# vinayak-gholap1993/Geometric-Multigrid-preconditioners-for-long-range-Coulomb-interaction

Hardware: AMD Instinct MI355X
Metric: DoF/s per CG-iter (GMG-precond Poisson, 3D) (higher is better)
Workload: dtype f64

## Files before the change

geometric-multigrid-preconditioners-for-long-range-coulomb-interaction_amd/capi.py:

```python
from __future__ import annotations

import ctypes as C
import os

import numpy as np

from . import build as _build

OK, ERR_INVALID, ERR_OUTER_NOCONV, ERR_COARSE_NOCONV, ERR_HIP, ERR_COMM, ERR_UNSUPPORTED = range(7)
SYSTEM = -1
JACOBI, SSOR, CHEBYSHEV = 0, 1, 2
PRECOND_GMG, PRECOND_JACOBI, PRECOND_IDENTITY = 0, 1, 2
SSOR_PARTITION_ROWS, SSOR_PARTITION_BALANCED = 0, 1
COARSE_CG, COARSE_DIRECT = 0, 1
CHEB_FIRST_KIND, CHEB_FOURTH_KIND = 0, 1
CHEB_LMAX_GERSHGORIN, CHEB_LMAX_LANCZOS = 0, 1
CHEBYSHEV_KEYS = ("polynomial", "lmax_source", "lanczos_steps", "steps_run", "gershgorin", "ritz", "safety", "lmax")
LEVEL_A, LEVEL_EDGE, LEVEL_EDGE_T = 0, 1, 2
UNIQUE_ID_BYTES = 128

SYMBOLS = [
    "gmg_create", "gmg_destroy", "gmg_reset", "gmg_last_error", "gmg_synchronize",
    "gmg_set_system_matrix", "gmg_set_level_matrix", "gmg_set_level_matrix_lattice", "gmg_set_edge_matrix", "gmg_set_prolongation", "gmg_build_transfer", "gmg_get_transfer",
    "gmg_assemble_system_matrix", "gmg_get_system_matrix", "gmg_system_matrix_norms",
    "gmg_assemble_level_matrix", "gmg_get_level_matrix", "gmg_assemble_system_matrix_coef", "gmg_assemble_level_matrix_coef",
    "gmg_assemble_rhs", "gmg_distribute_constraints",
    "gmg_build_mesh_tables", "gmg_get_mesh_tables", "gmg_get_mesh_level_tables",
    "gmg_close_constraints", "gmg_get_closed_constraints",
    "gmg_assemble_system_matrix_resident", "gmg_assemble_system_matrix_coef_resident", "gmg_assemble_level_matrix_resident",
    "gmg_assemble_level_matrix_coef_resident", "gmg_assemble_rhs_resident", "gmg_distribute_constraints_resident",
    "gmg_refine_forest", "gmg_get_refined_forest", "gmg_transfer_solution", "gmg_build_face_table",
    "gmg_estimate_error",
    "gmg_build_face_table_resident", "gmg_get_face_table", "gmg_estimate_error_resident", "gmg_get_marks", "gmg_refine_forest_marked",
    "gmg_energy_norm_error_resident",
    "gmg_build_point_locator_resident", "gmg_get_point_locator", "gmg_atom_forces_resident", "gmg_electrostatic_energy_resident",
    "gmg_set_copy_indices", "gmg_set_smoother", "gmg_set_coarse", "gmg_set_chebyshev", "gmg_estimate_lmax", "gmg_get_chebyshev",
    "gmg_set_coarse_solver", "gmg_coarse_direct_tables", "gmg_coarse_direct_separable", "gmg_coarse_direct_transform", "gmg_coarse_direct_profile",
    "gmg_vec_alloc", "gmg_vec_free", "gmg_vec_upload", "gmg_vec_download", "gmg_vec_set_zero", "gmg_vec_equ",
    "gmg_vec_add", "gmg_vec_sadd", "gmg_vec_dot", "gmg_vec_norms", "gmg_vec_all_zero",
    "gmg_spmv", "gmg_precondition", "gmg_precondition_jacobi", "gmg_coarse_solve", "gmg_smoother_step",
    "gmg_prolongate", "gmg_restrict_and_add", "gmg_cg_solve", "gmg_cg_direction_step", "gmg_cg_update_step",
    "gmg_comm_unique_id", "gmg_comm_init", "gmg_comm_barrier", "gmg_comm_info", "gmg_set_halo_plan", "gmg_set_global_sizes", "gmg_partition_range",
    "gmg_vec_allgather",
    "gmg_stats_reset", "gmg_stats_get", "gmg_set_profiling", "gmg_set_tuning", "gmg_set_option", "gmg_set_ssor_blocks",
    "gmg_set_ssor_block_rows", "gmg_set_ssor_partition", "gmg_get_ssor_partition", "gmg_ssor_balance_rows", "gmg_calibrate_hbm", "gmg_charge_density", "gmg_get_charge_density", "gmg_rhs_assemble",
    "gmg_charge_density_resident", "gmg_get_resident_cell_geometry",
    "gmg_set_point_locator", "gmg_atom_forces", "gmg_direct_coulomb",
    "gmg_gaussian_potential", "gmg_energy_norm_error",
    "gmg_get_ssor_plan", "gmg_get_ssor_backward_rows", "gmg_ssor_slot_plan",
    "gmg_get_ssor_plan_array", "gmg_get_ssor_plan_origin",
]


class Stats(C.Structure):
    _fields_ = [("coarse_solves", C.c_int64), ("coarse_iterations", C.c_int64), ("vcycles", C.c_int64),
                ("spmv0_samples", C.c_int64), ("spmv0_ms_total", C.c_double), ("spmv0_rows", C.c_int64),
                ("spmv0_nnz", C.c_int64), ("cgupd_samples", C.c_int64), ("cgupd_ms_total", C.c_double),
                ("coarse_variant", C.c_int64), ("spmv0_layout", C.c_int64), ("spmv0_matrix_bytes", C.c_int64),
                ("spmv0_pattern_slices", C.c_int64), ("spmv0_slices", C.c_int64), ("coarse_enqueued", C.c_int64),
                ("spmv0_noop_samples", C.c_int64), ("spmv0_noop_ms_total", C.c_double),
                ("sgs_samples", C.c_int64), ("sgs_ms_total", C.c_double), ("sgs_substeps", C.c_int64), ("sgs_stream_bytes", C.c_int64),
                ("sgs_launches", C.c_int64), ("build_matrices_ms", C.c_double), ("coarse_solver", C.c_int64)]


class GMGError(RuntimeError):
    def __init__(self, code, msg):
        super().__init__(f"gmg error {code}: {msg}")
        self.code = code


_lib = None


def load(build_if_missing: bool = False):
    global _lib
    if _lib is None:
        path = os.environ.get("GMG_DEVICE_LIB") or _build.LIB_DEVICE
        if build_if_missing:
            _build.build_device()
        if not os.path.exists(path):
            raise FileNotFoundError(f"{path} missing: run __graft_entry__.build() (hipcc --offload-arch=gfx950)")
        _lib = C.CDLL(path)
        _lib.gmg_last_error.restype = C.c_char_p
        _lib.gmg_last_error.argtypes = [C.c_void_p]
    return _lib


def _p(a, t):
    return a.ctypes.data_as(C.POINTER(t))


def _csr(m):
    return (np.ascontiguousarray(m.rowptr, dtype=np.int64), np.ascontiguousarray(m.col, dtype=np.int32),
            np.ascontiguousarray(m.val, dtype=np.float64))


class DeviceVector:
    def __init__(self, ctx: "Context", n: int):
        self.ctx, self.n = ctx, int(n)
        self.ptr = C.POINTER(C.c_double)()
        ctx._chk(ctx.L.gmg_vec_alloc(ctx.h, C.c_int64(self.n), C.byref(self.ptr)))

    def upload(self, a):
        a = np.ascontiguousarray(a, dtype=np.float64)
        assert a.size == self.n
        self.ctx._chk(self.ctx.L.gmg_vec_upload(self.ctx.h, self.ptr, _p(a, C.c_double), C.c_int64(self.n)))
        return self

    def download(self):
        out = np.empty(self.n)
        self.ctx._chk(self.ctx.L.gmg_vec_download(self.ctx.h, _p(out, C.c_double), self.ptr, C.c_int64(self.n)))
        return out

    def free(self):
        if self.ptr:
            self.ctx.L.gmg_vec_free(self.ctx.h, self.ptr)
            self.ptr = C.POINTER(C.c_double)()


class Context:

    def __init__(self, n_levels: int, device: int = 0):
        self.L = load()
        self.h = C.c_void_p()
        rc = self.L.gmg_create(C.byref(self.h), C.c_int(device), C.c_int(n_levels))
        if rc != OK:
            raise GMGError(rc, "gmg_create failed (no MI355X visible?)")
        self.n_levels = n_levels
        self.n_system = 0

    @classmethod
    def view(cls, handle):
        self = cls.__new__(cls)
# ... 789 lines not shown
    def synchronize(self):
        self._chk(self.L.gmg_synchronize(self.h))

    @staticmethod
    def unique_id() -> bytes:
        buf = C.create_string_buffer(UNIQUE_ID_BYTES)
        rc = load().gmg_comm_unique_id(buf)
        if rc != OK:
            raise GMGError(rc, "gmg_comm_unique_id failed")
        return buf.raw

    def comm_init(self, rank, n_ranks, uid: bytes):
        buf = C.create_string_buffer(uid, UNIQUE_ID_BYTES)
        self._chk(self.L.gmg_comm_init(self.h, C.c_int(rank), C.c_int(n_ranks), buf))

    def comm_barrier(self):
        self._chk(self.L.gmg_comm_barrier(self.h))

    def comm_info(self) -> dict:
        out = (C.c_int64 * 8)()
        self._chk(self.L.gmg_comm_info(self.h, out))
        return {"ranks": int(out[0]), "transport": {0: "none", 1: "rccl", 2: "peer"}[int(out[1])], "mailbox_finegrained": bool(out[2]),
                "ring_memory": {-1: "not allocated", 0: "hipMalloc (coarse-grained)", 1: "fine-grained"}[int(out[3])],
                "devices": int(out[4]), "level0_partitioned": bool(out[5])}

    def set_global_sizes(self, n_system, n_level0):
        self._chk(self.L.gmg_set_global_sizes(self.h, C.c_int64(n_system), C.c_int64(n_level0)))

    def allgather(self, n_global, dst_full, src_local):
        self._chk(self.L.gmg_vec_allgather(self.h, C.c_int64(n_global), dst_full.ptr, src_local.ptr))

    def set_halo_plan(self, which, neighbor_rank, send_count, send_idx, recv_count):
        nr = np.ascontiguousarray(neighbor_rank, dtype=np.int32)
        sc = np.ascontiguousarray(send_count, dtype=np.int32)
        si = np.ascontiguousarray(send_idx, dtype=np.int32)
        rc_ = np.ascontiguousarray(recv_count, dtype=np.int32)
        self._chk(self.L.gmg_set_halo_plan(self.h, C.c_int(which), C.c_int(len(nr)), _p(nr, C.c_int32), _p(sc, C.c_int32),
                                           _p(si, C.c_int32), _p(rc_, C.c_int32)))

    def stats(self) -> Stats:
        s = Stats()
        self._chk(self.L.gmg_stats_get(self.h, C.byref(s)))
        return s

    def stats_reset(self):
        self._chk(self.L.gmg_stats_reset(self.h))

    def set_profiling(self, every):
        self._chk(self.L.gmg_set_profiling(self.h, C.c_int(every)))

    def calibrate_hbm(self, n_bytes=1 << 30, reps=10):
        r, c = C.c_double(0), C.c_double(0)
        self._chk(self.L.gmg_calibrate_hbm(self.h, C.c_int64(n_bytes), C.c_int(reps), C.byref(r), C.byref(c)))
        return r.value, c.value

    def set_tuning(self, coarse_chunk=0, cg_variant=0, ssor_blocks=0):
        self._chk(self.L.gmg_set_tuning(self.h, C.c_int(coarse_chunk), C.c_int(cg_variant)))
        if ssor_blocks:
            self._chk(self.L.gmg_set_ssor_blocks(self.h, C.c_int(ssor_blocks)))

    def set_option(self, key: str, value: float = 1.0):
        self._chk(self.L.gmg_set_option(self.h, key.encode(), C.c_double(value)))

    def set_ssor_block_rows(self, level, block_row):
        b = np.ascontiguousarray(block_row, dtype=np.int64)
        n_blocks = max(len(b) - 1, 0)
        self._chk(self.L.gmg_set_ssor_block_rows(self.h, C.c_int(level), C.c_int(n_blocks), _p(b, C.c_int64) if len(b) else None))

    def set_ssor_partition(self, kind):
        self._chk(self.L.gmg_set_ssor_partition(self.h, C.c_int(kind)))

    def get_ssor_partition(self, level):
        nb = C.c_int(0)
        self._chk(self.L.gmg_get_ssor_partition(self.h, C.c_int(level), C.byref(nb), None, None))
        br, st = np.zeros(nb.value + 1, dtype=np.int64), np.zeros(max(nb.value, 1), dtype=np.int64)
        self._chk(self.L.gmg_get_ssor_partition(self.h, C.c_int(level), C.byref(nb), _p(br, C.c_int64), _p(st, C.c_int64)))
        return br, st[:nb.value]

    def get_ssor_plan(self, level):
        out = np.zeros(8, dtype=np.int64)
        self._chk(self.L.gmg_get_ssor_plan(self.h, C.c_int(level), _p(out, C.c_int64)))
        return dict(zip(SSOR_PLAN_KEYS, (int(v) for v in out)))

    def get_ssor_backward_rows(self, level):
        cnt = C.c_int64(0)
        self._chk(self.L.gmg_get_ssor_backward_rows(self.h, C.c_int(level), C.byref(cnt), None))
        rows = np.zeros(max(cnt.value, 1), dtype=np.int32)
        self._chk(self.L.gmg_get_ssor_backward_rows(self.h, C.c_int(level), C.byref(cnt), _p(rows, C.c_int32)))
        return rows[:cnt.value]

    def get_ssor_plan_array(self, level, which):
        w = SSOR_PLAN_ARRAYS.index(which) if isinstance(which, str) else int(which)
        nbytes = C.c_int64(0)
        self._chk(self.L.gmg_get_ssor_plan_array(self.h, C.c_int(level), C.c_int(w), C.byref(nbytes), None))
        out = np.zeros(max(nbytes.value, 1), dtype=np.uint8)
        self._chk(self.L.gmg_get_ssor_plan_array(self.h, C.c_int(level), C.c_int(w), C.byref(nbytes), out.ctypes.data_as(C.c_void_p)))
        return out[:nbytes.value]

    def get_ssor_plan_origin(self, level):
        on_dev, moved, why = C.c_int(0), C.c_int64(0), C.c_char_p()
        self._chk(self.L.gmg_get_ssor_plan_origin(self.h, C.c_int(level), C.byref(on_dev), C.byref(moved), C.byref(why)))
        return bool(on_dev.value), int(moved.value), (why.value or b"").decode()


SSOR_PLAN_ARRAYS = ("stream", "ranges", "blk_tab", "block_rng", "row_ci", "ci_row", "rpos_f", "rpos_b", "iso_diag", "iso_invd")
SSOR_PLAN_KEYS = ("forward_ranges", "backward_ranges", "self_contained_ranges", "y_slots", "max_live_forward", "max_live_backward", "steps", "stream_bytes")


def ssor_slot_plan(m, row_begin, row_end, backward):
    rp, col, val = _csr(m)
    n = len(rp) - 1
    k = max(int(row_end) - int(row_begin), 1)
    step, last, slot = (np.full(k, -1, dtype=np.int32) for _ in range(3))
    ns, nl = C.c_int64(0), C.c_int64(0)
    rc = load().gmg_ssor_slot_plan(C.c_int64(n), _p(rp, C.c_int64), _p(col, C.c_int32), _p(val, C.c_double), C.c_int64(int(row_begin)), C.c_int64(int(row_end)),
                                   C.c_int(int(bool(backward))), _p(step, C.c_int32), _p(last, C.c_int32), _p(slot, C.c_int32), C.byref(ns), C.byref(nl))
    if rc != OK:
        raise GMGError(rc, "gmg_ssor_slot_plan")
    k = int(row_end) - int(row_begin)
    return step[:k], last[:k], slot[:k], ns.value, nl.value


def ssor_balance_rows(m, n_blocks, use_values=True):
    rp, col, val = _csr(m)
    n = len(rp) - 1
    br, cost = np.zeros(n_blocks + 1, dtype=np.int64), np.zeros(n_blocks)
    rc = load().gmg_ssor_balance_rows(C.c_int64(n), _p(rp, C.c_int64), _p(col, C.c_int32), _p(val, C.c_double) if use_values else None,
                                      C.c_int(n_blocks), _p(br, C.c_int64), _p(cost, C.c_double))
    if rc != OK:
        raise GMGError(rc, "gmg_ssor_balance_rows")
    return br, cost


def coarse_direct_tables(n_cells):
    m = int(n_cells) - 1
    S, lam, mu = np.zeros((max(m, 1), max(m, 1))), np.zeros(max(m, 1)), np.zeros(max(m, 1))
    rc = load().gmg_coarse_direct_tables(C.c_int(int(n_cells)), _p(S, C.c_double), _p(lam, C.c_double), _p(mu, C.c_double))
    if rc != OK:
        raise GMGError(rc, "gmg_coarse_direct_tables")
    return S, lam, mu


def coarse_direct_separable(Ke):
    ke = np.ascontiguousarray(Ke, dtype=np.float64).reshape(64)
    s = C.c_double(0)
    rc = load().gmg_coarse_direct_separable(_p(ke, C.c_double), C.byref(s))
    if rc == ERR_UNSUPPORTED:
        return None
    if rc != OK:
        raise GMGError(rc, "gmg_coarse_direct_separable")
    return s.value
```

geometric-multigrid-preconditioners-for-long-range-coulomb-interaction_amd/csrc/gmg_coulomb.hip:

```cpp
#include "../../include/gmg_coulomb.h"
#include "gmg_device.hpp"
#include "gmg_sgs_layout.hpp"
#include "gmg_sgs.hpp"
#include "gmg_sgs_phase.hpp"
#include "gmg_sgs_dep.hpp"
#include "gmg_sgs_reg.hpp"
#include "gmg_sgs_plan.hpp"
#ifdef GMG_EXPERIMENTS
#include "gmg_sgs_chain.hpp"
#endif
#include "gmg_lattice.hpp"
#include "gmg_transfer.hpp"
#include "gmg_forces.hpp"
#include "gmg_exact.hpp"
#include "gmg_assemble.hpp"
#include "gmg_rhs_cells.hpp"
#include "gmg_estimate.hpp"
#include "gmg_fastdiag.hpp"
#include "gmg_lanczos.hpp"
#include "gmg_mesh_tables.hpp"
#include "gmg_close.hpp"
#include "gmg_refine.hpp"
#include "gmg_density.hpp"
#include "gmg_mem.hpp"
#include <hip/hip_ext.h>

#include <algorithm>
#include <array>
#include <chrono>
#include <cmath>
#include <cstdio>
#include <cstdlib>
#include <cstring>
#include <climits>
#include <map>
#include <queue>
#include <string>
#include <thread>
#include <unordered_map>
#include <vector>

#include "gmg_comm.hpp"

using namespace gmg;

namespace {

struct DevCSR {
  int64_t n_rows = 0, n_cols = 0, nnz = 0;
  DevPtr<int32_t> rowptr, col;
  DevPtr<double> val;
  DevPtr<int32_t> tile_row;
  int n_tiles = 0, tiles_per_xcd = 0, grid = 0;
  bool valid = false;
  HaloPlan halo;
  bool sell = false;
  DevPtr<int32_t> slice_ptr;
  DevPtr<int32_t> slice_base;
  DevPtr<void> sell_vals;
  DevPtr<void> sell_cols;
  DevPtr<double> sell_dict;
  DevPtr<int32_t> sell_spat, sell_pat;
  int sellp_pid = -1, sellp_centre[9] = {};
  DevPtr<int32_t> sellp_wave_ptr;
  DevPtr<int4> sellp_wave_rr;
  bool use_sellp = false;
  bool rowclass = false;
  DevPtr<uint8_t> sellp_rowcls;
  DevPtr<double> sellp_ctab;
  int n_classes = 0;
  int n_patterns = 0, n_pattern_slices = 0;
  bool val8 = false, col16 = false;
  int n_slices = 0, sell_grid = 0;
  int64_t sell_quads = 0;
  bool lattice = false;
  DevPtr<uint8_t> lat_rowcls;
  DevPtr<double> lat_ctab;
  DevPtr<int32_t> lat_gen;
  bool lat_only = false;
  int lat_W = 0;
  int64_t lat_fast_rows = 0;
  int lat_classes = 0, lat_nx = 0, lat_nxy = 0, lat_R0 = 0, lat_R1 = 0, lat_C = 0, lat_K = 0, lat_S = 0, lat_fast_blocks = 0, lat_n_gen = 0, lat_grid = 0;
  int64_t lat_gen_bytes = 0;
  bool hyb = false, hyb_val8 = false;
  DevPtr<int32_t> hyb_qptr, hyb_spat, hyb_pat, hyb_tiles, hyb_reg;
  DevPtr<void> hyb_vals, hyb_cols;
  DevPtr<double> hyb_dict;
  int hyb_n_slices = 0, hyb_n_reg = 0, hyb_n_pattern_slices = 0, hyb_n_tiles = 0, hyb_tile_blocks = 0, hyb_grid = 0;
  int64_t hyb_stream_bytes = 0, hyb_csr_bytes = 0;
  int lat_nv[3] = {0, 0, 0};
  double lat_Ke[64] = {};
};

struct SgsPlan {
  DevPtr<int32_t> stage_ptr, stage_rows, block_row, block_stage;
  int n_blocks = 0;
  int n_stages_max = 0;
  bool wave = false;
  DevPtr<SwRange> w_ranges;
  DevPtr<int32_t> w_block_rng, w_ws_ci, w_ci_row, w_row_ci, w_rpos_f, w_rpos_b;
  DevPtr<char> w_stream;
  DevPtr<double> w_ycur, w_iso_diag, w_iso_invd;
  int w_y_slots = 0, w_lds_bytes = 0, w_n_ranges = 0;
  int n_bwd = 0;
  std::vector<int32_t> host_bwd_rows;
  int n_self = 0, live_max[2] = {0, 0};
  int64_t w_n_coupled = 0, w_stream_bytes = 0, w_steps = 0, w_stages = 0;
  std::vector<int32_t> host_block_row;
  std::vector<int64_t> host_block_steps;
  std::vector<int64_t> host_block_bytes;
  std::vector<int32_t> host_block_rng;
  DevPtr<double> w_stage;
  int64_t w_stage_len = 0;
  bool phased = false;
  bool dep = false;
  bool reg = false;
  DevPtr<PhRange> p_ranges;
  DevPtr<uint4> p_blk_tab;
  std::vector<PhRange> host_pranges;
  bool on_device = false;
  int64_t csr_bytes_down = 0;
  const char *host_reason = "";
};

struct Level {
  DevCSR A, I, It, P, Pt;
  bool has_I = false, has_P = false;
  int64_t n = 0;
  int64_t n_vec = 0;
  int64_t n_copy = 0;
  DevPtr<int32_t> copy_g, copy_l;
  std::vector<int32_t> host_copy_g, host_copy_l;
  int copy_version = 0;
  DevPtr<double> sol, def, t, w1, w2, w3;
  double *sol_full = nullptr, *def_full = nullptr;
  DevPtr<double> sol_full_own, def_full_own;
  DevPtr<double> invd;
  double cheb_lmax = 0.0;
  struct ChebEstimate {
    bool valid = false;
    int steps_run = 0;
    double ritz = 0.0;
  } cheb_est;
  SgsPlan sgs;
};

struct FastDiag {
  bool ready = false;
  double s = 0.0;
  int m[3] = {0, 0, 0}, ld[3] = {0, 0, 0};
  DevPtr<double> S[3], lam[3], mu[3];
  DevPtr<double> t1, t2;
};

struct MeshTables {
  bool valid = false;
  int dim = 0;
  int64_t n_cells = 0, n_dofs = 0, n_hanging = 0, n_lines = 0, n_entries = 0;
  DevPtr<int32_t> cell_dofs, constraint_of_dof, line_ptr, line_master, line_dof;
  DevPtr<uint8_t> cell_level;
  DevPtr<unsigned long long> vertex_of_dof;
  DevPtr<double> line_weight;
  struct PerLevel {
    int64_t n_cells = 0, n_dofs = 0;
    DevPtr<int32_t> cell_dofs;
    DevPtr<unsigned long long> vertex_of_dof;
    DevPtr<uint8_t> dof_flags;
  };
  std::vector<PerLevel> level;
  struct Closed {
    bool valid = false;
    int64_t n_entries = 0;
    int max_line = 0;
    bool any_inhom = false;
    DevPtr<int32_t> line_ptr, line_master;
    DevPtr<double> line_weight, line_inhom;
  } closed;
  struct Faces {
    bool valid = false;
    DevPtr<uint8_t> kind;
    DevPtr<int32_t> cell;
  } faces;
  struct Marks {
    bool valid = false;
    int64_t n_marked = 0;
    DevPtr<uint8_t> mark;
  } marks;
  struct PointLocator {
    bool valid = false;
    int64_t n_nodes = 0;
    int32_t n0[3] = {0, 0, 0};
    DevPtr<int32_t> node;
  } locator;
};

struct RefinedForest {
  bool valid = false;
  int n_levels = 0;
  int64_t n_cells = 0, n_flags = 0, n_split = 0;
  std::vector<int64_t> level_ptr;
  DevPtr<int32_t> coord, first_child, parent;
  DevPtr<uint8_t> closed;
};

}

struct gmg_context {
  int device = 0;
  hipStream_t stream = nullptr;
  int n_levels = 0;
  std::vector<Level> lv;
  DevCSR S;
  DevPtr<double> S_invd;
  DevPtr<double> S_tmp;
  int smoother = GMG_SMOOTHER_SSOR;
  double omega = 0.5;
  int steps = 2;
  int cheb_degree = 2;
  double cheb_ratio = 30.0, cheb_lmax_user = 0.0;
  int cheb_polynomial = GMG_CHEB_FIRST_KIND, cheb_lmax_source = GMG_CHEB_LMAX_GERSHGORIN, cheb_lanczos_steps = 10;
  double cheb_safety = 1.2;
  int cheb_degree_opt = 0;
  int lanczos_max_blocks = 0;
  double coarse_tol = 1e-10;
  int coarse_maxit = 1000;
  int coarse_solver = GMG_COARSE_CG;
  bool coarse_direct_opt = false;
  int coarse_direct_max_blocks = 0;
  FastDiag fd;
  int64_t cg_n = 0;
  DevPtr<double> cg_g, cg_d0, cg_d1, cg_h;
  double *cg_ring[kXRing] = {};
  DevPtr<double> cg_ring_own[kXRing];
  int64_t cg_ring_len = 0;
  char *ring_shared[kPeerMaxRanks] = {};
  int64_t ring_stride = 0;
  int64_t peer_meta[kPeerMaxRanks][4 + kPeerMaxRanks] = {};
  unsigned long long peer_tag0 = 1;
  DevPtr<unsigned int> peer_push_cnt;
  DevPtr<CGState> st;
  HostPtr<CGState> st_host;
  CGState st_final{};
  Event ev_chunk[2];
  DevPtr<double> part_a, part_b;
  DevPtr<double> lanczos_rec;
  DevPtr<double> scal_dev;
  HostPtr<double> scal_host;
  DevPtr<double> ocg_dev;
  int ocg_cur = 0;
  double ocg_gh = 0.0;
  bool disable_vcycle_fused = false;
  DevPtr<int32_t> mgcopy_to, mgcopy_from_level, mgcopy_from_row;
  std::vector<int64_t> mgcopy_sig;
  bool mgcopy_ok = false;
  bool hybrid_two_launches = false;
  bool disable_hybrid = false;
  bool disable_outer_cg_fused = false;
  HostPtr<int> sgs_abort;
  int coarse_chunk = 0;
  int sgs_y_slots = 0;
  bool ssor_plan_device = false;
  bool sgs_sliding = true;
  bool sgs_disable_wave = false, sgs_disable_phase = false, sgs_chain = false, sgs_dep = false, sgs_reg = false, debug_upload = false, sgs_profile = false;
  int sgs_profile_mode = 0;
  int sgs_phase_chunk = 0;
  int sgs_pf_lead_kb = 0;
  bool sgs_phase_nocascade = false;
  bool sgs_phase_nosplit = false;
  int sgs_phase_profile = 0;
  int sgs_groups = 0;
  int sgs_lds_bytes_override = 0;
  bool disable_sell = false, disable_patterns = false, disable_compression = false, disable_sellp = false, disable_rowclass = false, disable_lattice = false;
  int lattice_segments = 0;
  int lattice_max_blocks = 0;
  int sell_grid = 0;
  int sellp_rr = 0;
  double sellp_cost = 4.0;
  int ssor_blocks = 1;
  int ssor_partition = GMG_SSOR_PARTITION_ROWS;
  std::map<int, std::vector<int64_t>> ssor_block_rows;
  int cg_variant = 0;
  int last_coarse_iters = 0;
  int prof_every = 0;
  std::vector<Event> ev_a, ev_b;
  std::vector<Event> ev_c, ev_d;
  std::vector<Event> ev_e, ev_f;
  bool launch_refused = false;
  int ev_used = 0, ev2_used = 0, ev3_used = 0;
  long long sgs_launch_no = 0;
  hipEvent_t timed_start = nullptr, timed_stop = nullptr;
  gmg_stats stats{};
  DevPtr<double> dens_dev;
  int64_t dens_cells = 0;
  int dens_nq = 0;
  gmg_forces::Locator loc{};
  DevPtr<int32_t> loc_node, loc_dofs;
  int64_t loc_max_dof = -1;
  int force_block = 64;
  int exact_chunk_log2 = 35;
  bool reset_keeps_mesh_tables = false;
  int assemble_max_blocks = 0;
  MeshTables mesh;
  RefinedForest refined;
  int density_segment = 0;
  int estimate_max_blocks = 0;
  Comm comm;
  bool dist = false;
  int64_t sys_global = 0, l0_global = 0;
  DevPtr<double> sys_full_a, sys_full_b;
  std::string err;
};

namespace {

#define HIPC(call)                                                                                   \
  do {                                                                                               \
    hipError_t e_ = (call);                                                                          \
    if (e_ != hipSuccess) {                                                                          \
      ctx->err = std::string(#call) + ": " + hipGetErrorString(e_);                                  \
      return GMG_ERR_HIP;                                                                            \
    }                                                                                                \
  } while (0)

#define CHK(call)                 \
  do {                            \
    int rc_ = (call);             \
    if (rc_ != GMG_OK) return rc_; \
  } while (0)

#define RETURN_LAUNCHED(ctx)                                                      \
  do {                                                                            \
    const hipError_t e_ = hipGetLastError();                                      \
    if (e_ != hipSuccess) {                                                       \
      (ctx)->err = std::string("kernel launch: ") + hipGetErrorString(e_);       \
      return GMG_ERR_HIP;                                                         \
    }                                                                             \
    return GMG_OK;                                                                \
  } while (0)

int launch_status(gmg_context *ctx) {
  if (ctx->launch_refused) { ctx->launch_refused = false; return GMG_ERR_UNSUPPORTED; }
  RETURN_LAUNCHED(ctx);
}

int fail(gmg_context *ctx, int code, const char *msg) {
// ... 958 lines not shown
  if (fused) {
    for (int l = 0; l < ctx->n_levels; ++l) mc.sol[l] = (l == 0) ? ctx->lv[0].sol_full : ctx->lv[(size_t)l].sol.get();
    if (n_sys > 0) hipLaunchKernelGGL(mg_copy_from_kernel, dim3(grid_for(n_sys)), dim3(kThreads), 0, ctx->stream, mc);
  } else {
    HIPC(hipMemsetAsync(dst_v, 0, sizeof(double) * (size_t)n_sys, ctx->stream));
  }
  for (int l = 0; l < ctx->n_levels && !fused; ++l) {
    Level &L = ctx->lv[(size_t)l];
    const double *sol = (l == 0) ? L.sol_full : L.sol.get();
    if (L.n_copy)
      hipLaunchKernelGGL(gather_scatter_kernel, dim3(grid_for(L.n_copy)), dim3(kThreads), 0, ctx->stream, dst_v,
                         (const int32_t *)L.copy_g.get(), sol, (const int32_t *)L.copy_l.get(), L.n_copy);
  }
  if (ctx->dist) {
    int64_t b, e;
    part_range(ctx->sys_global, ctx->comm.rank, ctx->comm.n_ranks, &b, &e);
    if (e > b) HIPC(hipMemcpyAsync(dst, dst_v + b, sizeof(double) * (size_t)(e - b), hipMemcpyDeviceToDevice, ctx->stream));
  }
  ctx->stats.vcycles++;
  return launch_status(ctx);
}

int setup_diag(gmg_context *ctx, int64_t n, const int64_t *rp, const int32_t *col, const double *val, DevPtr<double> &invd_dev,
               double *lmax_out) {
  std::vector<double> invd((size_t)std::max<int64_t>(n, 1));
  double lmax = 0.0;
  for (int64_t i = 0; i < n; ++i) {
    double aii = 0.0, rs = 0.0;
    for (int64_t k = rp[i]; k < rp[i + 1]; ++k) {
      if (col[k] == i) aii = val[k];
      rs += std::fabs(val[k]);
    }
    invd[(size_t)i] = 1.0 / aii;
    lmax = std::max(lmax, rs / std::fabs(aii));
  }
  if (lmax_out) *lmax_out = lmax;
  CHK(alloc_vec(ctx, invd_dev, n));
  if (n) HIPC(hipMemcpyAsync(invd_dev.get(), invd.data(), sizeof(double) * (size_t)n, hipMemcpyHostToDevice, ctx->stream));
  HIPC(hipStreamSynchronize(ctx->stream));
  return GMG_OK;
}


int sgs_wave_tail(gmg_context *ctx, SgsPlan &G, bool ph, bool dep, bool reg) {
  HIPC(hipFuncSetAttribute((const void *)sgs_wave_kernel<false>, hipFuncAttributeMaxDynamicSharedMemorySize, 160 * 1024));
  HIPC(hipFuncSetAttribute((const void *)sgs_wave_kernel<true>, hipFuncAttributeMaxDynamicSharedMemorySize, 160 * 1024));
  HIPC(hipFuncSetAttribute((const void *)sgs_phase_kernel, hipFuncAttributeMaxDynamicSharedMemorySize, 160 * 1024));
  HIPC(hipFuncSetAttribute((const void *)sgs_phase_profile_kernel, hipFuncAttributeMaxDynamicSharedMemorySize, 160 * 1024));
  HIPC(hipFuncSetAttribute((const void *)sgs_dep_kernel, hipFuncAttributeMaxDynamicSharedMemorySize, 160 * 1024));
  HIPC(hipFuncSetAttribute((const void *)sgs_regs_kernel, hipFuncAttributeMaxDynamicSharedMemorySize, 160 * 1024));
#ifdef GMG_EXPERIMENTS
  HIPC(hipFuncSetAttribute((const void *)sgs_chain_kernel, hipFuncAttributeMaxDynamicSharedMemorySize, 160 * 1024));
#endif
  hipFuncAttributes fa{};
  HIPC(hipFuncGetAttributes(&fa, ph ? (const void *)sgs_phase_kernel : (const void *)sgs_wave_kernel<false>));
  G.wave = fa.sharedSizeBytes == 0;
  if (ph) {
    HIPC(hipFuncGetAttributes(&fa, (const void *)sgs_phase_profile_kernel));
    G.wave = G.wave && fa.sharedSizeBytes == 0;
  }
  if (dep) {
    HIPC(hipFuncGetAttributes(&fa, (const void *)sgs_dep_kernel));
    G.wave = G.wave && fa.sharedSizeBytes == 0;
  }
  if (reg) {
    HIPC(hipFuncGetAttributes(&fa, (const void *)sgs_regs_kernel));
    G.wave = G.wave && fa.sharedSizeBytes == 0;
  }
#ifdef GMG_EXPERIMENTS
  if (ph) {
    HIPC(hipFuncGetAttributes(&fa, (const void *)sgs_chain_kernel));
    G.wave = G.wave && fa.sharedSizeBytes == 0;
  }
#endif
  return GMG_OK;
}

SsorPlanOptions ssor_plan_options(const gmg_context *ctx) {
  SsorPlanOptions o;
  o.disable_wave = ctx->sgs_disable_wave; o.disable_phase = ctx->sgs_disable_phase; o.profile = ctx->sgs_profile;
  o.dep = ctx->sgs_dep; o.reg = ctx->sgs_reg; o.chain = ctx->sgs_chain; o.sliding = ctx->sgs_sliding;
  o.y_slots = ctx->sgs_y_slots; o.groups = ctx->sgs_groups; o.phase_chunk = ctx->sgs_phase_chunk;
  o.phase_nosplit = ctx->sgs_phase_nosplit; o.phase_nocascade = ctx->sgs_phase_nocascade; o.pf_lead_kb = ctx->sgs_pf_lead_kb;
  o.debug = ctx->debug_upload;
  return o;
}

static_assert(sizeof(PhBlkEntry) == sizeof(uint4) && alignof(PhBlkEntry) <= alignof(uint4), "the block table is read as uint4 by the sweep kernels");

void sgs_set_host_members(SgsPlan &G, const SsorSweepPlan &W, const std::vector<int32_t> &block_row, int64_t n_coupled, int64_t stream_bytes) {
  G.host_bwd_rows = W.bwd_rows; G.host_pranges = W.pranges;
  G.host_block_row = block_row; G.host_block_rng = W.block_rng; G.host_block_steps = W.block_steps; G.host_block_bytes = W.block_bytes;
  G.n_self = W.n_self; G.live_max[0] = W.live_max[0]; G.live_max[1] = W.live_max[1];
  G.w_y_slots = W.y_slots; G.w_lds_bytes = W.lds_bytes; G.w_n_ranges = W.n_ranges(); G.n_bwd = W.n_bwd;
  G.phased = W.phased; G.dep = W.dep; G.reg = W.reg;
  G.w_n_coupled = n_coupled; G.w_stream_bytes = stream_bytes; G.w_steps = W.total_steps; G.w_stages = W.total_stages;
}

void sgs_plan_log(const SgsPlan &G, const SsorSweepPlan &W, int64_t n) {
  const std::vector<int64_t> &hist_g = W.hist_g, &hist_l1 = W.hist_l1, &hist_l2 = W.hist_l2;
  if (W.phased)
    std::fprintf(stderr, "[gmg] SGS step shapes: G %lld %lld %lld %lld | L1/4 %lld %lld %lld %lld %lld %lld %lld %lld | L2/8 %lld %lld %lld %lld\n", (long long)hist_g[0], (long long)hist_g[1],
                 (long long)hist_g[2], (long long)hist_g[3], (long long)hist_l1[0], (long long)hist_l1[1], (long long)hist_l1[2], (long long)hist_l1[3], (long long)hist_l1[4],
                 (long long)hist_l1[5], (long long)hist_l1[6], (long long)hist_l1[7], (long long)hist_l2[0], (long long)hist_l2[1], (long long)hist_l2[2], (long long)hist_l2[3]);
  std::fprintf(stderr, "[gmg] SGS %s plan: %lld rows, %lld coupled, %d blocks, %lld stages, %lld sub-steps, %d ranges (%d forward + %d backward, %d self-contained), "
               "y slots %d (most live: forward %d, backward %d), stream %.1f MB\n",
               W.phased ? "four-wave" : "one-wave", (long long)n, (long long)G.w_n_coupled, (int)G.host_block_row.size() - 1, (long long)G.w_stages, (long long)G.w_steps, G.w_n_ranges,
               G.w_n_ranges - G.n_bwd, G.n_bwd, G.n_self, G.w_y_slots, G.live_max[0], G.live_max[1], (double)G.w_stream_bytes / 1e6);
}

void sgs_partition_log(gmg_context *ctx, Level &L, int64_t n, const int64_t *rp, const int32_t *col, const double *val, const std::vector<int32_t> &block_row,
                     bool explicit_rows) {
  const int n_blocks = (int)block_row.size() - 1;
  const std::vector<double> cost = ssor_block_costs(SsorPattern(n, rp, col, val), block_row);
  double c_max = 0, c_sum = 0;
  int64_t s_max = 0, s_sum = 0;
  for (int b = 0; b < n_blocks; ++b) {
    std::fprintf(stderr, "[gmg]   SSOR block %3d: rows [%lld, %lld) %lld, sub-steps %lld, stream %.2f MB, model %.1f us\n", b, (long long)block_row[(size_t)b],
                 (long long)block_row[(size_t)b + 1], (long long)(block_row[(size_t)b + 1] - block_row[(size_t)b]), (long long)L.sgs.host_block_steps[(size_t)b],
                 (double)L.sgs.host_block_bytes[(size_t)b] / 1e6, cost[(size_t)b]);
    c_max = std::max(c_max, cost[(size_t)b]); c_sum += cost[(size_t)b];
    s_max = std::max(s_max, L.sgs.host_block_steps[(size_t)b]); s_sum += L.sgs.host_block_steps[(size_t)b];
  }
  std::fprintf(stderr, "[gmg]   SSOR partition (%s): %d blocks, longest / mean: model %.2f, sub-steps %.2f\n",
               explicit_rows ? "caller's" : ctx->ssor_partition == GMG_SSOR_PARTITION_BALANCED ? "balanced" : "equal rows", n_blocks,
               c_sum > 0 ? c_max * n_blocks / c_sum : 1.0, s_sum > 0 ? (double)s_max * n_blocks / (double)s_sum : 1.0);
  if (L.sgs.w_stage.get()) {
    const int n_ranks = ctx->comm.n_ranks;
    std::fprintf(stderr, "[gmg]   SSOR all-gather: %d ranks x %lld doubles (largest piece) = %.2f MB moved per sweep for %.2f MB of y\n", n_ranks,
                 (long long)L.sgs.w_stage_len, 8e-6 * (double)L.sgs.w_stage_len * n_ranks, 8e-6 * (double)n);
  }
}

int setup_sgs(gmg_context *ctx, Level &L, int64_t n, const int64_t *rp, const int32_t *col, const double *val,
              const std::vector<int64_t> *explicit_rows) {
  const SsorPlanOptions opt = ssor_plan_options(ctx);
  const std::vector<int32_t> block_row = ssor_block_rows(n, rp, col, val, explicit_rows, ctx->ssor_partition == GMG_SSOR_PARTITION_BALANCED, ctx->ssor_blocks);
  const int n_blocks = (int)block_row.size() - 1;
  const SsorGenericPlan GP = ssor_generic_plan(n, rp, col, block_row);
  SsorSweepPlan W;
  ssor_sweep_plan(opt, n, rp, col, val, block_row, true, W);
  if (W.outcome == kSsorOneWave) ssor_sweep_plan(opt, n, rp, col, val, block_row, false, W);
  const auto t_planned = std::chrono::steady_clock::now();
  if (W.outcome == kSsorPlanned)
    if (const char *bad = check_sweep_plan(W, n)) { W.outcome = kSsorInvalid; W.message = bad; }
  const bool wave = W.outcome == kSsorPlanned;
  L.sgs = SgsPlan();
  SgsPlan &G = L.sgs;
  G.n_blocks = n_blocks; G.n_stages_max = GP.n_stages_max;
  HIPC(upload(G.stage_ptr, GP.stage_ptr, ctx->stream));
  HIPC(upload(G.stage_rows, GP.stage_rows, ctx->stream));
  HIPC(upload(G.block_row, block_row, ctx->stream));
  HIPC(upload(G.block_stage, GP.block_stage, ctx->stream));
  if (wave) {
    HIPC(upload(G.w_ranges, W.ranges, ctx->stream));
    HIPC(upload(G.p_ranges, W.pranges, ctx->stream));
    HIPC(upload(G.p_blk_tab, reinterpret_cast<const uint4 *>(W.blk_tab.data()), W.blk_tab.size(), ctx->stream));
    HIPC(upload(G.w_block_rng, W.block_rng, ctx->stream));
    HIPC(upload(G.w_ws_ci, W.ws_ci, ctx->stream));
    HIPC(upload(G.w_ci_row, W.ci_row, ctx->stream));
    HIPC(upload(G.w_row_ci, W.row_ci, ctx->stream));
    HIPC(upload(G.w_rpos_f, W.rpos_f, ctx->stream));
    HIPC(upload(G.w_rpos_b, W.rpos_b, ctx->stream));
    HIPC(upload(G.w_stream, W.stream, ctx->stream));
    HIPC(upload(G.w_iso_diag, W.iso_diag, ctx->stream));
    HIPC(upload(G.w_iso_invd, W.iso_invd, ctx->stream));
    if (!(W.phased && W.n_self == (int)W.pranges.size())) HIPC(G.w_ycur.alloc(std::max<size_t>(W.ci_row.size(), 1)));
  }
  HIPC(hipStreamSynchronize(ctx->stream));
  G.host_block_row = block_row;
  G.host_block_steps.assign((size_t)n_blocks, 0);
  for (int b = 0; b < n_blocks; ++b) G.host_block_steps[(size_t)b] = 2 * (int64_t)(GP.block_stage[(size_t)b + 1] - GP.block_stage[(size_t)b]);
  G.host_block_bytes.assign((size_t)n_blocks, 0);
  if (W.outcome == kSsorUnsupported || W.outcome == kSsorInvalid) return fail(ctx, W.outcome == kSsorUnsupported ? GMG_ERR_UNSUPPORTED : GMG_ERR_INVALID, W.message);
  if (wave) {
    if (ctx->debug_upload)
      std::fprintf(stderr, "[gmg] SGS plan laps (host, %lld rows): block graph %.4f s, steps + slots %.4f s, shapes %.4f s, record fill %.4f s, upload %.4f s\n", (long long)n,
                   W.laps[0], W.laps[1], W.laps[2], W.laps[3], std::chrono::duration<double>(std::chrono::steady_clock::now() - t_planned).count());
    sgs_set_host_members(G, W, block_row, (int64_t)W.ci_row.size(), (int64_t)W.stream.size());
    const int n_ranks = ctx->dist ? ctx->comm.n_ranks : 1;
    if (n_ranks > 1 && n_blocks % n_ranks == 0) {
      const int nbl = n_blocks / n_ranks;
      int64_t len = 1;
      for (int r = 0; r < n_ranks; ++r) len = std::max<int64_t>(len, block_row[(size_t)((r + 1) * nbl)] - block_row[(size_t)(r * nbl)]);
      G.w_stage_len = len;
      HIPC(G.w_stage.alloc((size_t)(len * n_ranks)));
    }
    CHK(sgs_wave_tail(ctx, G, W.phased, W.dep, W.reg));
    if (ctx->debug_upload) sgs_plan_log(G, W, n);
  }
  if (ctx->debug_upload) sgs_partition_log(ctx, L, n, rp, col, val, block_row, explicit_rows != nullptr);
  return GMG_OK;
}

dim3 asm_blocks(const gmg_context *ctx, int64_t n, int per_block, int most = 1 << 16) {
  int64_t g = std::max<int64_t>(1, std::min<int64_t>(most, (n + per_block - 1) / per_block));
  if (ctx->assemble_max_blocks > 0) g = std::min<int64_t>(g, ctx->assemble_max_blocks);
  return dim3((unsigned)g);
}

const char *sgs_device_refusal(const gmg_context *ctx, bool explicit_rows) {
  if (ctx->dist) return "communicator";
  if (!explicit_rows && ctx->ssor_partition == GMG_SSOR_PARTITION_BALANCED) return "balanced partition";
  if (!ctx->sgs_sliding) return "option sgs_sliding unset";
  if (ctx->sgs_disable_wave) return "option sgs_disable_wave set";
  if (ctx->sgs_disable_phase) return "option sgs_disable_phase set";
  if (ctx->sgs_profile) return "option sgs_profile set";
  if (ctx->sgs_dep) return "option sgs_dep set";
  if (ctx->sgs_reg) return "option sgs_reg set";
  if (ctx->sgs_chain) return "option sgs_chain set";
  if (ctx->sgs_groups) return "option sgs_groups set";
  if (ctx->sgs_phase_chunk) return "option sgs_phase_chunk set";
  if (ctx->sgs_phase_nosplit) return "option sgs_phase_nosplit set";
  if (ctx->sgs_phase_nocascade) return "option sgs_phase_nocascade set";
  if (ctx->sgs_pf_lead_kb) return "option sgs_pf_lead_kb set";
  return nullptr;
}

int setup_sgs_device(gmg_context *ctx, Level &L, int64_t n, const int32_t *rp, const int32_t *col, const double *val,
                     const std::vector<int64_t> *explicit_rows, const char **reason) {
  *reason = sgs_device_refusal(ctx, explicit_rows != nullptr);
  if (*reason) return GMG_OK;
  if (n <= 0) { *reason = "empty level"; return GMG_OK; }
  const std::vector<int32_t> block_row = ssor_block_rows(n, nullptr, nullptr, nullptr, explicit_rows, false, ctx->ssor_blocks);
  const int n_blocks = (int)block_row.size() - 1;
  int y_cap = ctx->sgs_y_slots > 0 ? ctx->sgs_y_slots : kPhYSlots;
  y_cap = std::max(64, std::min(y_cap, kPhYSlots)) & ~1;
  hipStream_t st = ctx->stream;
  const size_t N = (size_t)n, NB = (size_t)n_blocks;
  double laps[4] = {0, 0, 0, 0};
  auto lap_t = std::chrono::steady_clock::now();
  auto lap = [&](int k) {
    const auto t = std::chrono::steady_clock::now();
    laps[k] += std::chrono::duration<double>(t - lap_t).count();
    lap_t = t;
  };
  auto grid = [&](int64_t cnt) { return asm_blocks(ctx, cnt, 256); };
  auto scan = [&](int32_t *p, int64_t cnt) { hipLaunchKernelGGL(tr_scan_kernel, dim3(1), dim3(1024), 0, st, p, cnt); };
  sp::Args a{};
  a.n = n; a.n_blocks = n_blocks; a.y_cap = y_cap; a.rp = rp; a.col = col; a.val = val;
  DevPtr<int32_t> d_brow, d_prp, d_indeg, d_upptr, d_upfill, d_ccnt, d_stage, d_pcol, d_uplist, d_row_ci;
  DevPtr<uint8_t> d_coupled;
  DevPtr<uint32_t> d_flags;
  DevPtr<double> d_pval, d_iso_diag, d_iso_invd;
  DevPtr<sp::Block> d_blk;
  HIPC(upload(d_brow, block_row, st));
  HIPC(d_prp.alloc(N + 1)); HIPC(d_indeg.alloc(N)); HIPC(d_upptr.alloc(N + 1)); HIPC(d_upfill.alloc(N)); HIPC(d_ccnt.alloc(NB));
  HIPC(d_stage.alloc(N)); HIPC(d_coupled.alloc(N)); HIPC(d_flags.alloc(1)); HIPC(d_iso_diag.alloc(N)); HIPC(d_iso_invd.alloc(N)); HIPC(d_row_ci.alloc(N));
  HIPC(hipMemsetAsync(d_indeg.get(), 0, 4 * N, st)); HIPC(hipMemsetAsync(d_upptr.get(), 0, 4 * (N + 1), st)); HIPC(hipMemsetAsync(d_upfill.get(), 0, 4 * N, st));
  HIPC(hipMemsetAsync(d_ccnt.get(), 0, 4 * NB, st)); HIPC(hipMemsetAsync(d_coupled.get(), 0, N, st)); HIPC(hipMemsetAsync(d_flags.get(), 0, 4, st));
  HIPC(hipMemsetAsync(d_row_ci.get(), 0xff, 4 * N, st));
  a.brow = d_brow.get(); a.prp = d_prp.get(); a.indeg = d_indeg.get(); a.upptr = d_upptr.get(); a.upfill = d_upfill.get(); a.ccnt = d_ccnt.get();
  a.stage = d_stage.get(); a.coupled = d_coupled.get(); a.flags = d_flags.get(); a.iso_diag = d_iso_diag.get(); a.iso_invd = d_iso_invd.get(); a.row_ci = d_row_ci.get();
  hipLaunchKernelGGL(sp::graph_kernel<false>, grid(n), dim3(256), 0, st, a);
  hipLaunchKernelGGL(sp::coupled_count_kernel, grid(n), dim3(256), 0, st, a);
  scan(d_prp.get(), n);
  scan(d_upptr.get(), n);
  uint32_t flags = 0;
  int32_t n_pruned = 0, n_up = 0;
  std::vector<int32_t> ccnt(NB, 0);
  HIPC(hipMemcpyAsync(&flags, d_flags.get(), 4, hipMemcpyDeviceToHost, st));
  HIPC(hipMemcpyAsync(&n_pruned, d_prp.get() + n, 4, hipMemcpyDeviceToHost, st));
  HIPC(hipMemcpyAsync(&n_up, d_upptr.get() + n, 4, hipMemcpyDeviceToHost, st));
  HIPC(hipMemcpyAsync(ccnt.data(), d_ccnt.get(), 4 * NB, hipMemcpyDeviceToHost, st));
  HIPC(hipStreamSynchronize(st));
  CHK(launch_status(ctx));
  lap(0);
  if (flags & sp::kUnsorted) { *reason = "unsorted columns"; return GMG_OK; }
  if (flags & sp::kWide) { *reason = "row too wide"; return GMG_OK; }
  std::vector<sp::Block> blk(NB);
  SsorSweepPlan W;
  W.phased = true;
  std::vector<int32_t> &block_rng = W.block_rng;
  block_rng.assign(NB + 1, 0);
  int64_t nct = 0;
  for (int b = 0; b < n_blocks; ++b) {
    sp::Block &B = blk[(size_t)b];
    B = sp::Block{block_row[(size_t)b], block_row[(size_t)b + 1], (int32_t)nct, ccnt[(size_t)b], 0, 0, block_rng[(size_t)b], 0};
    nct += ccnt[(size_t)b];
    block_rng[(size_t)b + 1] = block_rng[(size_t)b] + (ccnt[(size_t)b] > 0 ? 2 : 0);
  }
  const int n_ranges = block_rng[NB];
  const size_t NC = (size_t)nct;
  a.n_coupled = (int32_t)nct;
  HIPC(upload(d_blk, blk, st));
  a.blk = d_blk.get();
  HIPC(d_pcol.alloc(std::max<size_t>((size_t)n_pruned, 1))); HIPC(d_pval.alloc(std::max<size_t>((size_t)n_pruned, 1))); HIPC(d_uplist.alloc(std::max<size_t>((size_t)n_up, 1)));
  a.pcol = d_pcol.get(); a.pval = d_pval.get(); a.uplist = d_uplist.get();
  hipLaunchKernelGGL(sp::graph_kernel<true>, grid(n), dim3(256), 0, st, a);
  DevPtr<int32_t> d_queue, d_sptr, d_stepbase, d_nstages, d_nsteps, d_ci_row, d_spos;
  HIPC(d_queue.alloc(std::max<size_t>(NC, 1))); HIPC(d_ci_row.alloc(std::max<size_t>(NC, 1)));
  HIPC(d_sptr.alloc(NC + NB + 1)); HIPC(d_stepbase.alloc(NC + NB + 1)); HIPC(d_spos.alloc(NC + NB + 1)); HIPC(d_nstages.alloc(NB)); HIPC(d_nsteps.alloc(NB));
  a.queue = d_queue.get(); a.ci_row = d_ci_row.get(); a.sptr = d_sptr.get(); a.spos = d_spos.get(); a.stepbase = d_stepbase.get(); a.nstages = d_nstages.get(); a.nsteps = d_nsteps.get();
  hipLaunchKernelGGL(sp::stage_kernel, asm_blocks(ctx, n_blocks, 1), dim3(1024), 0, st, a);
  std::vector<int32_t> nstages(NB, 0), nsteps(NB, 0);
  HIPC(hipMemcpyAsync(nstages.data(), d_nstages.get(), 4 * NB, hipMemcpyDeviceToHost, st));
  HIPC(hipMemcpyAsync(nsteps.data(), d_nsteps.get(), 4 * NB, hipMemcpyDeviceToHost, st));
  HIPC(hipMemcpyAsync(&flags, d_flags.get(), 4, hipMemcpyDeviceToHost, st));
  HIPC(hipStreamSynchronize(st));
  CHK(launch_status(ctx));
  lap(1);
  if (flags & sp::kInternal) return fail(ctx, GMG_ERR_INVALID, "SSOR plan on the device: the stage propagation did not reach every coupled row (internal error)");
  int64_t n_steps = 0, total_stages = 0;
  for (int b = 0; b < n_blocks; ++b) {
// ... 47 lines not shown
  W.block_steps.assign(NB, 0); W.block_bytes.assign(NB, 0);
  for (int b = 0; b < n_blocks; ++b) {
    const sp::Block &B = blk[(size_t)b];
    if (B.nc == 0) continue;
    W.block_steps[(size_t)b] = 2 * (int64_t)B.S;
    const int64_t bytes0 = stream_size;
    for (int dir = 1; dir >= 0; --dir) {
      const int ns = nslots[2 * (size_t)b + dir];
      live_max[dir] = std::max(live_max[dir], ns);
      max_ws = std::max(max_ws, ns);
      PhRange P{};
      P.backward = dir; P.pad0[0] = 1; P.pad0[1] = ns;
      P.n_steps = B.S;
      const int64_t base = (stream_size + 1023) / 1024 * 1024, off = (int64_t)rbytes[2 * (size_t)b + dir] * 16;
      P.stream_off = base;
      P.blk_tab = (uint32_t)(B.g0 + (dir ? 0 : B.S));
      const int64_t padded = (off + 2048 + 1023) / 1024 * 1024;
      if (padded >= ((int64_t)1 << 31) || (base + padded) / 8 >= ((int64_t)1 << 31)) { *reason = "stream positions beyond 2^31"; return GMG_OK; }
      P.stream_bytes = (uint32_t)padded;
      stream_size = base + padded;
      pranges[(size_t)(B.rng + dir)] = P;
      rbase[(size_t)(B.rng + dir)] = base;
    }
    W.block_bytes[(size_t)b] = stream_size - bytes0;
  }
  const int y_slots = std::max(2, (max_ws + 1) & ~1);
  DevPtr<int64_t> d_rbase;
  DevPtr<char> d_stream;
  DevPtr<uint4> d_blk_tab;
  DevPtr<PhRange> d_pranges;
  DevPtr<int32_t> d_rpos, d_block_rng;
  DevPtr<unsigned long long> d_chk;
  HIPC(upload(d_rbase, rbase, st));
  HIPC(upload(d_pranges, pranges, st));
  HIPC(upload(d_block_rng, block_rng, st));
  HIPC(d_stream.alloc(std::max<size_t>((size_t)stream_size, 1))); HIPC(d_blk_tab.alloc(std::max<size_t>(NS, 1))); HIPC(d_rpos.alloc(std::max<size_t>(2 * NC, 1))); HIPC(d_chk.alloc(8));
  HIPC(hipMemsetAsync(d_stream.get(), 0, std::max<size_t>((size_t)stream_size, 1), st));
  HIPC(hipMemsetAsync(d_chk.get(), 0, 64, st));
  a.rbase = d_rbase.get(); a.stream = d_stream.get(); a.blk_tab = d_blk_tab.get(); a.rpos = d_rpos.get();
  if (nct > 0) {
    hipLaunchKernelGGL(sp::record_kernel, grid(2 * nct), dim3(256), 0, st, a);
    hipLaunchKernelGGL(sp::header_kernel, grid(n_steps), dim3(256), 0, st, a);
  }
  sp::CheckArgs c{};
  c.ranges = d_pranges.get(); c.blk_tab = d_blk_tab.get(); c.stream = d_stream.get(); c.rpos_f = d_rpos.get(); c.rpos_b = d_rpos.get() + NC;
  c.n_ranges = n_ranges; c.n_coupled = (int32_t)nct; c.y_slots = y_slots; c.stream_bytes = stream_size; c.out = d_chk.get();
  hipLaunchKernelGGL(sp::check_kernel, asm_blocks(ctx, std::max(n_ranges, 1), 1, 1024), dim3(256), 0, st, c);
  unsigned long long chk[8] = {};
  std::vector<int32_t> ci_row(NC);
  std::vector<uint4> blk_tab_h;
  HIPC(hipMemcpyAsync(chk, d_chk.get(), 64, hipMemcpyDeviceToHost, st));
  if (NC) HIPC(hipMemcpyAsync(ci_row.data(), d_ci_row.get(), 4 * NC, hipMemcpyDeviceToHost, st));
  if (ctx->debug_upload && NS) {
    blk_tab_h.resize(NS);
    HIPC(hipMemcpyAsync(blk_tab_h.data(), d_blk_tab.get(), 16 * NS, hipMemcpyDeviceToHost, st));
  }
  HIPC(hipStreamSynchronize(st));
  CHK(launch_status(ctx));
  if (chk[0]) return fail(ctx, GMG_ERR_INVALID, "SSOR plan on the device: the block table, a header or a record fails the plan's checks (internal error)");
  if (stream_size > 0 && (chk[1] * 8 + 8 > (uint64_t)stream_size || chk[2] + 8 > (uint64_t)y_slots * 8))
    return fail(ctx, GMG_ERR_INVALID, "SSOR plan on the device: a record addresses memory outside the stream / the LDS slots (internal error)");
  if (chk[3] >= (uint64_t)n) return fail(ctx, GMG_ERR_INVALID, "SSOR plan on the device: a backward record stores outside the level vector (internal error)");
  if (NC && chk[4] * 8 + 8 > (uint64_t)stream_size) return fail(ctx, GMG_ERR_INVALID, "SSOR plan on the device: rhs position outside the stream (internal error)");
  L.sgs = SgsPlan();
  SgsPlan &G = L.sgs;
  G.n_blocks = n_blocks;
  HIPC(upload(G.w_ranges, std::vector<SwRange>(), st));
  HIPC(upload(G.w_ws_ci, std::vector<int32_t>(), st));
  G.p_ranges = std::move(d_pranges); G.p_blk_tab = std::move(d_blk_tab); G.w_block_rng = std::move(d_block_rng);
  G.w_ci_row = std::move(d_ci_row); G.w_row_ci = std::move(d_row_ci); G.w_stream = std::move(d_stream);
  G.w_iso_diag = std::move(d_iso_diag); G.w_iso_invd = std::move(d_iso_invd);
  HIPC(G.w_rpos_f.alloc(std::max<size_t>(NC, 1))); HIPC(G.w_rpos_b.alloc(std::max<size_t>(NC, 1)));
  if (NC) {
    HIPC(hipMemcpyAsync(G.w_rpos_f.get(), d_rpos.get(), 4 * NC, hipMemcpyDeviceToDevice, st));
    HIPC(hipMemcpyAsync(G.w_rpos_b.get(), d_rpos.get() + NC, 4 * NC, hipMemcpyDeviceToDevice, st));
  }
  HIPC(hipStreamSynchronize(st));
  for (int b = 0; b < n_blocks; ++b)
    for (int q = blk[(size_t)b].nc - 1; q >= 0; --q) W.bwd_rows.push_back(ci_row[(size_t)(blk[(size_t)b].q0 + q)]);
  W.n_self = n_ranges; W.n_bwd = n_ranges / 2;
  W.y_slots = y_slots;
  W.lds_bytes = y_slots * 8 + kPhWaves * kPhRegion + kPhJunk;
  W.total_steps = n_steps; W.total_stages = total_stages;
  sgs_set_host_members(G, W, block_row, nct, stream_size);
  G.on_device = true;
  CHK(sgs_wave_tail(ctx, G, true, false, false));
  if (!G.wave) return fail(ctx, GMG_ERR_INVALID, "SSOR plan on the device: the sweep kernel has static LDS (internal error)");
  lap(3);
  if (ctx->debug_upload) {
    std::fprintf(stderr, "[gmg] SGS plan laps (device, %lld rows): graph %.4f s, stages %.4f s, order + slots + shapes + offsets %.4f s, records + check %.4f s\n", (long long)n,
                 laps[0], laps[1], laps[2], laps[3]);
    for (const uint4 &e : blk_tab_h) {
      int g, l1, l2;
      sp::key_shape((int)(e.z & 255u), &g, &l1, &l2);
      W.hist_l1[(size_t)std::min(7, l1 / 4)]++; W.hist_l2[(size_t)(l2 / 8)]++; W.hist_g[(size_t)g]++;
    }
    sgs_plan_log(G, W, n);
  }
  return GMG_OK;
}

template <class Fetch>
int setup_sgs_any(gmg_context *ctx, Level &L, int64_t n, const int32_t *d_rp, const int32_t *d_col, const double *d_val, const int64_t *rp64,
                  const int32_t *col, const double *val, const std::vector<int64_t> *explicit_rows, Fetch fetch) {
  const char *reason = "";
  int64_t moved = 0;
  if (ctx->ssor_plan_device) {
    CHK(setup_sgs_device(ctx, L, n, d_rp, d_col, d_val, explicit_rows, &reason));
    if (!reason) {
      if (ctx->debug_upload) {
        if (!col) CHK(fetch(&col, &val, &moved));
        L.sgs.csr_bytes_down = moved;
        sgs_partition_log(ctx, L, n, rp64, col, val, L.sgs.host_block_row, explicit_rows != nullptr);
      }
      return GMG_OK;
    }
  }
  if (!col) CHK(fetch(&col, &val, &moved));
  CHK(setup_sgs(ctx, L, n, rp64, col, val, explicit_rows));
  L.sgs.csr_bytes_down = moved;
  L.sgs.host_reason = reason;
  return GMG_OK;
}

void free_cg_ring(gmg_context *ctx) {
  if (ctx->ring_shared[ctx->comm.rank]) comm_share_free(ctx->comm, ctx->ring_shared);
  for (int r = 0; r < kXRing; ++r) { ctx->cg_ring[r] = nullptr; ctx->cg_ring_own[r].reset(); }
  ctx->cg_ring_len = 0;
}

void free_locator(gmg_context *ctx) {
  ctx->loc_node.reset(); ctx->loc_dofs.reset();
  ctx->loc = gmg_forces::Locator{};
  ctx->loc_max_dof = -1;
}

void release_operators(gmg_context *ctx) {
  for (auto &L : ctx->lv) L = Level();
  ctx->S = DevCSR();
  for (DevPtr<double> *p : {&ctx->sys_full_a, &ctx->sys_full_b, &ctx->S_invd, &ctx->S_tmp, &ctx->cg_g, &ctx->cg_d0, &ctx->cg_d1, &ctx->cg_h}) p->reset();
  free_cg_ring(ctx);
  drop_coarse_direct(ctx);
}

int tile_device_csr(gmg_context *ctx, DevCSR &m, const std::vector<int32_t> &rp, int64_t n_rows, int64_t n_cols, int64_t nnz) {
  const TilePlan T = plan_tiles(rp.data(), n_rows);
  m.n_rows = n_rows; m.n_cols = n_cols; m.nnz = nnz;
  set_tiles(m, T);
  HIPC(upload(m.tile_row, T.tile_row, ctx->stream));
  HIPC(hipStreamSynchronize(ctx->stream));
  CHK(launch_status(ctx));
  m.valid = true;
  return GMG_OK;
}

struct AsmScratch {
  DevPtr<int32_t> iptr, ipos, islot;
  DevPtr<unsigned long long> total;
  DevPtr<int> over;
};

template <bool LEVEL>
int assemble_incidence(gmg_context *ctx, AsmArgs &a, AsmScratch &w, int32_t &n_inc) {
  const int64_t n_dofs = a.n_dofs, n_slots = a.n_slots;
  HIPC(w.iptr.alloc((size_t)n_dofs + 1));
  HIPC(w.ipos.alloc((size_t)n_dofs + 1));
// ... 213 lines not shown
int gmg_set_system_matrix(gmg_context *ctx, int64_t n_rows, int64_t n_cols, const int64_t *rowptr, const int32_t *col,
                          const double *val) {
  if (!ctx) return GMG_ERR_INVALID;
  (void)hipSetDevice(ctx->device);
  CHK(upload_csr(ctx, ctx->S, n_rows, n_cols, rowptr, col, val, false, true));
  CHK(setup_diag(ctx, n_rows, rowptr, col, val, ctx->S_invd, nullptr));
  CHK(alloc_vec(ctx, ctx->S_tmp, n_cols));
  if (ctx->dist) {
    const int64_t padded = part_chunk(ctx->sys_global, ctx->comm.n_ranks) * ctx->comm.n_ranks;
    CHK(alloc_vec(ctx, ctx->sys_full_a, padded));
    CHK(alloc_vec(ctx, ctx->sys_full_b, padded));
    int64_t b, e;
    part_range(ctx->sys_global, ctx->comm.rank, ctx->comm.n_ranks, &b, &e);
    if (e - b != n_rows) return fail(ctx, GMG_ERR_INVALID, "system matrix rows do not match the canonical partition");
  }
  return GMG_OK;
}

static int finish_level(gmg_context *ctx, int level, int64_t n_rows, int64_t n_cols, int64_t nnz) {
  Level &L = ctx->lv[(size_t)level];
  L.n = n_rows;
  L.n_vec = n_cols;
  for (DevPtr<double> *p : {&L.sol, &L.def, &L.t, &L.w1, &L.w2, &L.w3}) CHK(alloc_vec(ctx, *p, n_cols));
  if (level == 0) {
    if (l0_partitioned(ctx)) {
      const int64_t padded = part_chunk(ctx->l0_global, ctx->comm.n_ranks) * ctx->comm.n_ranks;
      CHK(alloc_vec(ctx, L.sol_full_own, padded));
      CHK(alloc_vec(ctx, L.def_full_own, padded));
      L.sol_full = L.sol_full_own.get();
      L.def_full = L.def_full_own.get();
    } else {
      L.sol_full_own.reset(); L.def_full_own.reset();
      L.sol_full = L.sol.get();
      L.def_full = L.def.get();
    }
    ctx->cg_n = n_cols;
    for (DevPtr<double> *p : {&ctx->cg_g, &ctx->cg_d0, &ctx->cg_d1, &ctx->cg_h}) CHK(alloc_vec(ctx, *p, n_cols));
    free_cg_ring(ctx);
    ctx->stats.spmv0_rows = n_rows;
    ctx->stats.spmv0_nnz = nnz;
    ctx->stats.spmv0_layout = L.A.sell ? 1 + (L.A.val8 ? 2 : 0) + (L.A.col16 ? 4 : 0) + (L.A.use_sellp ? 8 : 0) : 0;
    if (L.A.sell) {
      const double frac_stream = L.A.n_slices ? 1.0 - (double)L.A.n_pattern_slices / L.A.n_slices : 1.0;
      const int64_t ent = L.A.sell_quads * 256;
      const int64_t val_bytes = L.A.rowclass ? (int64_t)(frac_stream * (double)ent) + (int64_t)L.A.n_pattern_slices * 64 : ent * (L.A.val8 ? 1 : 8);
      ctx->stats.spmv0_matrix_bytes = val_bytes + (int64_t)(frac_stream * (double)ent * (L.A.col16 ? 2 : 4)) + 8 * (int64_t)L.A.n_slices;
      if (L.A.rowclass) ctx->stats.spmv0_layout += 16;
      if (L.A.lattice) {
        ctx->stats.spmv0_layout += 32;
        ctx->stats.spmv0_matrix_bytes = L.A.lat_fast_rows + L.A.lat_gen_bytes;
      }
    } else if (L.A.lat_only) {
      ctx->stats.spmv0_layout = 1 + 2 + 4 + 8 + 16 + 32 + 64;
      ctx->stats.spmv0_matrix_bytes = n_rows;
    } else {
      ctx->stats.spmv0_matrix_bytes = 12 * nnz + 4 * (n_rows + 1);
    }
    ctx->stats.spmv0_pattern_slices = L.A.n_pattern_slices;
    ctx->stats.spmv0_slices = L.A.n_slices;
    ctx->last_coarse_iters = 0;
  }
  HIPC(hipStreamSynchronize(ctx->stream));
  return GMG_OK;
}

int gmg_set_level_matrix(gmg_context *ctx, int level, int64_t n_rows, int64_t n_cols, const int64_t *rowptr,
                         const int32_t *col, const double *val) {
  if (!ctx || level < 0 || level >= ctx->n_levels) return GMG_ERR_INVALID;
  const auto ex = level > 0 ? ctx->ssor_block_rows.find(level) : ctx->ssor_block_rows.end();
  const std::vector<int64_t> *explicit_rows = ex == ctx->ssor_block_rows.end() ? nullptr : &ex->second;
  if (explicit_rows && explicit_rows->back() != n_rows)
    return fail(ctx, GMG_ERR_INVALID, "gmg_set_level_matrix: the SSOR block boundaries of this level (gmg_set_ssor_block_rows) do not end at n_rows");
  (void)hipSetDevice(ctx->device);
  Level &L = ctx->lv[(size_t)level];
  if (level == 0) drop_coarse_direct(ctx);
  L.cheb_est = Level::ChebEstimate();
  CHK(upload_csr(ctx, L.A, n_rows, n_cols, rowptr, col, val, level > 0));
  CHK(setup_diag(ctx, n_rows, rowptr, col, val, L.invd, &L.cheb_lmax));
  if (level > 0) {
    L.n = n_rows;
    if (ctx->ssor_plan_device) {
      DevPtr<int32_t> d_rp, d_col;
      DevPtr<double> d_val;
      if (!sgs_device_refusal(ctx, explicit_rows != nullptr) && n_rows > 0) {
        if (rowptr[n_rows] > INT32_MAX) return fail(ctx, GMG_ERR_INVALID, "gmg_set_level_matrix: more than 2^31 entries");
        const std::vector<int32_t> rp32(rowptr, rowptr + n_rows + 1);
        HIPC(upload(d_rp, rp32, ctx->stream));
        HIPC(upload(d_col, col, (size_t)rowptr[n_rows], ctx->stream));
        HIPC(upload(d_val, val, (size_t)rowptr[n_rows], ctx->stream));
        HIPC(hipStreamSynchronize(ctx->stream));
      }
      const int rc_plan = setup_sgs_any(ctx, L, n_rows, d_rp.get(), d_col.get(), d_val.get(), rowptr, col, val, explicit_rows,
                                        [](const int32_t **, const double **, int64_t *) { return (int)GMG_OK; });
      if (rc_plan != GMG_OK) {
        reset_keep_halo(L.A);
        L.invd.reset();
        L.cheb_lmax = 0.0;
        L.cheb_est = Level::ChebEstimate();
        L.sgs = SgsPlan();
        return rc_plan;
      }
    } else {
      CHK(setup_sgs(ctx, L, n_rows, rowptr, col, val, explicit_rows));
    }
  }
  return finish_level(ctx, level, n_rows, n_cols, rowptr[n_rows]);
}

int gmg_set_level_matrix_lattice(gmg_context *ctx, int level, const int32_t nv[3], const double Ke[64]) {
  if (!ctx || !nv || !Ke || level < 0 || level >= ctx->n_levels) return GMG_ERR_INVALID;
  if (level != 0) return fail(ctx, GMG_ERR_UNSUPPORTED, "gmg_set_level_matrix_lattice: level 0 only (finer levels of an adaptive hierarchy are patches, and their smoothers need the rows)");
  if (l0_partitioned(ctx)) return fail(ctx, GMG_ERR_UNSUPPORTED, "gmg_set_level_matrix_lattice: a row-partitioned level 0 takes its local rows as CSR (gmg_set_level_matrix)");
  const int64_t nx = nv[0], ny = nv[1], nz = nv[2];
  if (nx < 5 || ny < 5 || nz < 5) return fail(ctx, GMG_ERR_INVALID, "gmg_set_level_matrix_lattice: at least 5 vertices per direction");
  const int64_t n = nx * ny * nz, nxy = nx * ny, reach = nxy + nx + 1;
  if (n >= ((int64_t)1 << 28)) return fail(ctx, GMG_ERR_UNSUPPORTED, "gmg_set_level_matrix_lattice: more than 2^28 rows");
  (void)hipSetDevice(ctx->device);
  Level &L = ctx->lv[0];
  DevCSR &m = L.A;
  drop_coarse_direct(ctx);
  reset_keep_halo(m);
  L.cheb_est = Level::ChebEstimate();
  for (int d = 0; d < 3; ++d) m.lat_nv[d] = nv[d];
  std::copy(Ke, Ke + 64, m.lat_Ke);
  const int64_t dims[3] = {nx, ny, nz};
  auto rep = [&](int t, int64_t mdim) -> int64_t { return t == 0 ? 0 : t == 1 ? 1 : t == 2 ? 2 : t == 3 ? mdim - 2 : mdim - 1; };
  std::vector<double> ctab((size_t)125 * 27, 0.0);
  double lmax = 0.0;
  for (int cls = 0; cls < 125; ++cls) {
    const int t[3] = {cls % 5, (cls / 5) % 5, cls / 25};
    int64_t v[3];
    bool v_bnd = false;
    for (int d = 0; d < 3; ++d) { v[d] = rep(t[d], dims[d]); v_bnd = v_bnd || v[d] == 0 || v[d] == dims[d] - 1; }
    double rowsum = 0.0;
    for (int j = 0; j < 27; ++j) {
      const int dd[3] = {j % 3 - 1, (j / 3) % 3 - 1, j / 9 - 1};
      int64_t u[3];
      bool exists = true, u_bnd = false;
      for (int d = 0; d < 3; ++d) {
        u[d] = v[d] + dd[d];
        exists = exists && u[d] >= 0 && u[d] < dims[d];
        u_bnd = u_bnd || u[d] == 0 || u[d] == dims[d] - 1;
      }
      double acc = 0.0;
      if (exists && ((v_bnd && j == 13) || (!v_bnd && !u_bnd))) {
        int64_t lo[3], hi[3];
        for (int d = 0; d < 3; ++d) { lo[d] = std::max<int64_t>(std::max(v[d], u[d]) - 1, 0); hi[d] = std::min<int64_t>(std::min(v[d], u[d]), dims[d] - 2); }
        for (int64_t cz = lo[2]; cz <= hi[2]; ++cz)
          for (int64_t cy = lo[1]; cy <= hi[1]; ++cy)
            for (int64_t cx = lo[0]; cx <= hi[0]; ++cx) {
              const int a = (int)((v[0] - cx) + 2 * (v[1] - cy) + 4 * (v[2] - cz)), b = (int)((u[0] - cx) + 2 * (u[1] - cy) + 4 * (u[2] - cz));
              acc += v_bnd ? std::fabs(Ke[a * 8 + a]) : Ke[a * 8 + b];
            }
      }
      ctab[(size_t)cls * 27 + (size_t)j] = acc;
      rowsum += std::fabs(acc);
    }
    lmax = std::max(lmax, rowsum / std::fabs(ctab[(size_t)cls * 27 + 13]));
  }
  LatticeClassMap cmap{};
  std::vector<double> utab;
  int n_unique = 0;
  for (int cls = 0; cls < 125; ++cls) {
    int found = -1;
    for (int q = 0; q < n_unique && found < 0; ++q)
      if (std::memcmp(&utab[(size_t)q * 27], &ctab[(size_t)cls * 27], sizeof(double) * 27) == 0) found = q;
    if (found < 0) {
// ... 2819 lines not shown
int gmg_stats_get(gmg_context *ctx, gmg_stats *out) {
  if (!ctx || !out) return GMG_ERR_INVALID;
  collect_sgs_samples(ctx);
  *out = ctx->stats;
  return GMG_OK;
}
int gmg_set_profiling(gmg_context *ctx, int sample_every) {
  if (!ctx || sample_every < 0) return GMG_ERR_INVALID;
  ctx->prof_every = sample_every;
  if (sample_every > 0 && ctx->ev_a.empty()) {
    for (auto *v : {&ctx->ev_a, &ctx->ev_b, &ctx->ev_c, &ctx->ev_d, &ctx->ev_e, &ctx->ev_f}) {
      v->resize(256);
      for (auto &e : *v) HIPC(e.create());
    }
  }
  return GMG_OK;
}
int gmg_calibrate_hbm(gmg_context *ctx, int64_t n_bytes, int reps, double *read_gbps, double *copy_gbps) {
  if (!ctx || n_bytes < (1 << 20) || reps < 1) return GMG_ERR_INVALID;
  const int64_t n2 = n_bytes / 16;
  DevPtr<double2> a_own, b_own;
  Event e0_own, e1_own;
  HIPC(a_own.alloc((size_t)n2));
  HIPC(b_own.alloc((size_t)n2));
  double2 *const a = a_own.get(), *const b = b_own.get();
  HIPC(hipMemsetAsync(a, 0, (size_t)n2 * 16, ctx->stream));
  HIPC(hipMemsetAsync(b, 0, (size_t)n2 * 16, ctx->stream));
  HIPC(e0_own.create());
  HIPC(e1_own.create());
  const hipEvent_t e0 = e0_own.get(), e1 = e1_own.get();
  float ms = 0.f;
  for (int pass = 0; pass < 2; ++pass) {
    HIPC(hipEventRecord(e0, ctx->stream));
    for (int r = 0; r < reps; ++r)
      hipLaunchKernelGGL(stream_read_kernel, dim3(kMaxPartials), dim3(kThreads), 0, ctx->stream, (const double2 *)a, n2, ctx->part_a.get());
    HIPC(hipEventRecord(e1, ctx->stream));
    HIPC(hipEventSynchronize(e1));
    HIPC(hipEventElapsedTime(&ms, e0, e1));
  }
  if (read_gbps) *read_gbps = (double)n2 * 16 * reps / (ms * 1e-3) / 1e9;
  for (int pass = 0; pass < 2; ++pass) {
    HIPC(hipEventRecord(e0, ctx->stream));
    for (int r = 0; r < reps; ++r)
      hipLaunchKernelGGL(stream_copy_kernel, dim3(kMaxPartials * 2), dim3(kThreads), 0, ctx->stream, (const double2 *)a, b, n2);
    HIPC(hipEventRecord(e1, ctx->stream));
    HIPC(hipEventSynchronize(e1));
    HIPC(hipEventElapsedTime(&ms, e0, e1));
  }
  if (copy_gbps) *copy_gbps = (double)n2 * 32 * reps / (ms * 1e-3) / 1e9;
  return GMG_OK;
}

int gmg_set_option(gmg_context *ctx, const char *key, double value) {
  if (!ctx || !key) return GMG_ERR_INVALID;
  const std::string k(key);
  const bool on = value != 0.0;
  if (k == "host_threads") g_host_threads = (int)value;
  else if (k == "debug_upload") ctx->debug_upload = on;
  else if (k == "disable_sell") ctx->disable_sell = on;
  else if (k == "disable_outer_cg_fused") ctx->disable_outer_cg_fused = on;
  else if (k == "disable_hybrid") ctx->disable_hybrid = on;
  else if (k == "hybrid_two_launches") ctx->hybrid_two_launches = on;
  else if (k == "disable_vcycle_fused") ctx->disable_vcycle_fused = on;
  else if (k == "disable_patterns") ctx->disable_patterns = on;
  else if (k == "disable_compression") ctx->disable_compression = on;
  else if (k == "disable_sellp") ctx->disable_sellp = on;
  else if (k == "disable_rowclass") ctx->disable_rowclass = on;
  else if (k == "disable_lattice") ctx->disable_lattice = on;
  else if (k == "lattice_segments") ctx->lattice_segments = (int)value;
  else if (k == "lattice_max_blocks") ctx->lattice_max_blocks = (int)value;
  else if (k == "sell_grid") ctx->sell_grid = (int)value;
  else if (k == "sellp_cost") ctx->sellp_cost = value;
  else if (k == "sellp_rr") ctx->sellp_rr = (int)value;
  else if (k == "cg_variant") ctx->cg_variant = (int)value;
  else if (k == "coarse_chunk") ctx->coarse_chunk = (int)value;
  else if (k == "coarse_direct") ctx->coarse_direct_opt = on;
  else if (k == "coarse_direct_max_blocks") {
    if (!(value >= 0 && value <= 65536) || value != (double)(int)value) return fail(ctx, GMG_ERR_INVALID, "coarse_direct_max_blocks: an integer in 0 .. 65536");
    ctx->coarse_direct_max_blocks = (int)value;
  }
  else if (k == "ssor_balanced") ctx->ssor_partition = on ? GMG_SSOR_PARTITION_BALANCED : GMG_SSOR_PARTITION_ROWS;
  else if (k == "sgs_y_slots") ctx->sgs_y_slots = (int)value;
  else if (k == "sgs_sliding") ctx->sgs_sliding = on;
  else if (k == "ssor_plan_device") ctx->ssor_plan_device = on;
  else if (k == "sgs_disable_wave") ctx->sgs_disable_wave = on;
  else if (k == "sgs_disable_phase") ctx->sgs_disable_phase = on;
  else if (k == "sgs_dep") ctx->sgs_dep = on;
  else if (k == "sgs_reg") ctx->sgs_reg = on;
  else if (k == "sgs_pf_lead_kb") ctx->sgs_pf_lead_kb = (int)value;
  else if (k == "sgs_chain") {
#ifndef GMG_EXPERIMENTS
    if (on) return fail(ctx, GMG_ERR_UNSUPPORTED, "sgs_chain needs a -DGMG_EXPERIMENTS build (tools/build_experiments.sh)");
#endif
    ctx->sgs_chain = on;
  }
  else if (k == "sgs_phase_profile") {
    if (on && ctx->dist && ctx->comm.n_ranks > 1) return fail(ctx, GMG_ERR_INVALID, "sgs_phase_profile: one rank only (the instrumented sweep is a single-GPU measurement)");
    ctx->sgs_phase_profile = (int)value;
  }
  else if (k == "sgs_phase_nosplit") ctx->sgs_phase_nosplit = on;
  else if (k == "sgs_phase_nocascade") ctx->sgs_phase_nocascade = on;
  else if (k == "sgs_phase_chunk") ctx->sgs_phase_chunk = (int)value;
  else if (k == "force_block") {
    if (value != 64 && value != 128 && value != 256) return fail(ctx, GMG_ERR_INVALID, "force_block: 64, 128 or 256");
    ctx->force_block = (int)value;
  }
  else if (k == "reset_keeps_mesh_tables") ctx->reset_keeps_mesh_tables = on;
  else if (k == "density_segment") {
    if (!(value >= 0 && value <= 2047) || value != (double)(int)value) return fail(ctx, GMG_ERR_INVALID, "density_segment: an integer in 0 .. 2047");
    ctx->density_segment = (int)value;
  } else if (k == "assemble_max_blocks") {
    if (!(value >= 0 && value <= 65536) || value != (double)(int)value) return fail(ctx, GMG_ERR_INVALID, "assemble_max_blocks: an integer in 0 .. 65536");
    ctx->assemble_max_blocks = (int)value;
  }
  else if (k == "estimate_max_blocks") {
    if (!(value >= 0 && value <= 65536) || value != (double)(int)value) return fail(ctx, GMG_ERR_INVALID, "estimate_max_blocks: an integer in 0 .. 65536");
    ctx->estimate_max_blocks = (int)value;
  }
  else if (k == "exact_chunk_log2") {
    if (!(value >= 0 && value <= 35) || value != (double)(int)value) return fail(ctx, GMG_ERR_INVALID, "exact_chunk_log2: an integer in 0 .. 35");
    ctx->exact_chunk_log2 = (int)value;
  }
  else if (k == "cheb_polynomial") {
    if (value != GMG_CHEB_FIRST_KIND && value != GMG_CHEB_FOURTH_KIND) return fail(ctx, GMG_ERR_INVALID, "cheb_polynomial: 0 (first kind) or 1 (fourth kind)");
    return gmg_set_chebyshev(ctx, (int)value, ctx->cheb_lmax_source, 0, 0.0);
  }
  else if (k == "cheb_lmax_source") {
    if (value != GMG_CHEB_LMAX_GERSHGORIN && value != GMG_CHEB_LMAX_LANCZOS) return fail(ctx, GMG_ERR_INVALID, "cheb_lmax_source: 0 (Gershgorin) or 1 (Lanczos)");
    return gmg_set_chebyshev(ctx, ctx->cheb_polynomial, (int)value, 0, 0.0);
  }
  else if (k == "cheb_lanczos_steps") {
    if (!(value >= 1 && value <= lanczos::kMaxSteps) || value != (double)(int)value) return fail(ctx, GMG_ERR_INVALID, "cheb_lanczos_steps: an integer in 1 .. 64");
    return gmg_set_chebyshev(ctx, ctx->cheb_polynomial, ctx->cheb_lmax_source, (int)value, 0.0);
  }
  else if (k == "cheb_safety") {
    if (!(value >= 1.0)) return fail(ctx, GMG_ERR_INVALID, "cheb_safety: a factor >= 1");
    return gmg_set_chebyshev(ctx, ctx->cheb_polynomial, ctx->cheb_lmax_source, 0, value);
  }
  else if (k == "cheb_degree") {
    if (!(value >= 0 && value <= 64) || value != (double)(int)value) return fail(ctx, GMG_ERR_INVALID, "cheb_degree: an integer in 0 .. 64 (0: the degree of gmg_set_smoother)");
    ctx->cheb_degree_opt = (int)value;
  }
  else if (k == "lanczos_max_blocks") {
    if (!(value >= 0 && value <= 65536) || value != (double)(int)value) return fail(ctx, GMG_ERR_INVALID, "lanczos_max_blocks: an integer in 0 .. 65536");
    ctx->lanczos_max_blocks = (int)value;
  }
  else if (k == "sgs_groups") ctx->sgs_groups = (int)value;
  else if (k == "sgs_lds_bytes_override") ctx->sgs_lds_bytes_override = (int)value;
  else if (k == "sgs_profile") {
    if (on && ctx->dist && ctx->comm.n_ranks > 1) return fail(ctx, GMG_ERR_INVALID, "sgs_profile: one rank only");
    ctx->sgs_profile = on;
    ctx->sgs_profile_mode = (int)value - 1;
#ifndef GMG_EXPERIMENTS
    if (ctx->sgs_profile_mode > 0) return fail(ctx, GMG_ERR_UNSUPPORTED, "sgs_profile modes > 1 need a -DGMG_EXPERIMENTS build (tools/build_experiments.sh)");
#endif
  }
  else return fail(ctx, GMG_ERR_INVALID, "gmg_set_option: unknown key");
  return GMG_OK;
}

int gmg_set_tuning(gmg_context *ctx, int coarse_chunk, int cg_variant) {
  if (!ctx || coarse_chunk < 0 || cg_variant < 0 || cg_variant > 2) return GMG_ERR_INVALID;
  ctx->coarse_chunk = coarse_chunk;
  ctx->cg_variant = cg_variant;
  return GMG_OK;
}

int gmg_set_ssor_blocks(gmg_context *ctx, int n_blocks) {
  if (!ctx || n_blocks < 1) return GMG_ERR_INVALID;
  ctx->ssor_blocks = n_blocks;
  return GMG_OK;
}

int gmg_set_ssor_block_rows(gmg_context *ctx, int level, int n_blocks, const int64_t *block_row) {
  if (!ctx) return GMG_ERR_INVALID;
  if (level < 1 || level >= ctx->n_levels) return fail(ctx, GMG_ERR_INVALID, "gmg_set_ssor_block_rows: levels 1 .. n_levels - 1 (level 0 is the coarse CG)");
  if (n_blocks < 0 || (n_blocks > 0 && !block_row)) return fail(ctx, GMG_ERR_INVALID, "gmg_set_ssor_block_rows: n_blocks >= 0 boundaries expected");
  if (n_blocks == 0) {
    ctx->ssor_block_rows.erase(level);
    return GMG_OK;
  }
  if (block_row[0] != 0) return fail(ctx, GMG_ERR_INVALID, "gmg_set_ssor_block_rows: the first boundary must be 0");
  for (int b = 0; b < n_blocks; ++b)
    if (block_row[b + 1] < block_row[b]) return fail(ctx, GMG_ERR_INVALID, "gmg_set_ssor_block_rows: boundaries must not decrease");
  if (block_row[n_blocks] > INT32_MAX) return fail(ctx, GMG_ERR_INVALID, "gmg_set_ssor_block_rows: rows beyond the 32-bit range");
  ctx->ssor_block_rows[level].assign(block_row, block_row + n_blocks + 1);
  return GMG_OK;
}

int gmg_set_ssor_partition(gmg_context *ctx, int kind) {
  if (!ctx) return GMG_ERR_INVALID;
  if (kind != GMG_SSOR_PARTITION_ROWS && kind != GMG_SSOR_PARTITION_BALANCED) return fail(ctx, GMG_ERR_INVALID, "gmg_set_ssor_partition: unknown kind");
  ctx->ssor_partition = kind;
  return GMG_OK;
}

int gmg_get_ssor_partition(gmg_context *ctx, int level, int *n_blocks, int64_t *block_row, int64_t *block_steps) {
  if (!ctx || !n_blocks || level < 1 || level >= ctx->n_levels) return GMG_ERR_INVALID;
  const SgsPlan &G = ctx->lv[(size_t)level].sgs;
  if (G.host_block_row.empty()) return fail(ctx, GMG_ERR_INVALID, "gmg_get_ssor_partition: the level matrix has not been set");
  *n_blocks = (int)G.host_block_row.size() - 1;
  if (block_row) std::copy(G.host_block_row.begin(), G.host_block_row.end(), block_row);
  if (block_steps) std::copy(G.host_block_steps.begin(), G.host_block_steps.end(), block_steps);
  return GMG_OK;
}

int gmg_ssor_balance_rows(int64_t n, const int64_t *rowptr, const int32_t *col, const double *val, int n_blocks, int64_t *block_row,
                          double *block_cost) {
  if (n < 0 || n > INT32_MAX || n_blocks < 1 || !block_row || (n > 0 && (!rowptr || !col)) || (n > 0 && rowptr[0] != 0)) return GMG_ERR_INVALID;
  for (int64_t i = 0; i < n; ++i) {
    if (rowptr[i + 1] < rowptr[i]) return GMG_ERR_INVALID;
    for (int64_t k = rowptr[i]; k < rowptr[i + 1]; ++k)
      if (col[k] < 0 || col[k] >= n) return GMG_ERR_INVALID;
  }
  std::vector<int64_t> br;
  std::vector<double> cost;
  if (n == 0) {
    br.assign((size_t)n_blocks + 1, 0);
    cost.assign((size_t)n_blocks, 0.0);
  } else {
    ssor_balance(SsorPattern(n, rowptr, col, val), n_blocks, br, cost);
  }
  std::copy(br.begin(), br.end(), block_row);
  if (block_cost) std::copy(cost.begin(), cost.end(), block_cost);
  return GMG_OK;
}

int gmg_get_ssor_plan(gmg_context *ctx, int level, int64_t out[8]) {
  if (!ctx || !out || level < 1 || level >= ctx->n_levels) return GMG_ERR_INVALID;
  const SgsPlan &G = ctx->lv[(size_t)level].sgs;
  if (G.host_block_row.empty()) return fail(ctx, GMG_ERR_INVALID, "gmg_get_ssor_plan: the level matrix has not been set");
  std::fill(out, out + 8, (int64_t)0);
  if (!G.wave) return GMG_OK;
  out[0] = G.w_n_ranges - G.n_bwd; out[1] = G.n_bwd; out[2] = G.n_self; out[3] = G.w_y_slots;
  out[4] = G.live_max[0]; out[5] = G.live_max[1]; out[6] = G.w_steps; out[7] = G.w_stream_bytes;
  return GMG_OK;
}

int gmg_get_ssor_backward_rows(gmg_context *ctx, int level, int64_t *count, int32_t *rows) {
  if (!ctx || !count || level < 1 || level >= ctx->n_levels) return GMG_ERR_INVALID;
  const SgsPlan &G = ctx->lv[(size_t)level].sgs;
  if (G.host_block_row.empty()) return fail(ctx, GMG_ERR_INVALID, "gmg_get_ssor_backward_rows: the level matrix has not been set");
  *count = G.wave ? (int64_t)G.host_bwd_rows.size() : 0;
  if (rows && G.wave) std::copy(G.host_bwd_rows.begin(), G.host_bwd_rows.end(), rows);
  return GMG_OK;
}

int gmg_get_ssor_plan_array(gmg_context *ctx, int level, int which, int64_t *bytes, void *out) {
  if (!ctx || !bytes || level < 1 || level >= ctx->n_levels) return GMG_ERR_INVALID;
  const Level &L = ctx->lv[(size_t)level];
  const SgsPlan &G = L.sgs;
  if (G.host_block_row.empty() || !G.wave || !G.phased) return fail(ctx, GMG_ERR_INVALID, "gmg_get_ssor_plan_array: the level has no four-wave plan");
  const void *src = nullptr;
  int64_t len = 0;
  switch (which) {
    case GMG_SSOR_PLAN_STREAM: src = G.w_stream.get(); len = G.w_stream_bytes; break;
    case GMG_SSOR_PLAN_RANGES: src = G.p_ranges.get(); len = (int64_t)sizeof(PhRange) * G.w_n_ranges; break;
    case GMG_SSOR_PLAN_BLK_TAB: src = G.p_blk_tab.get(); len = 16 * G.w_steps; break;
    case GMG_SSOR_PLAN_BLOCK_RNG: src = G.w_block_rng.get(); len = 4 * (int64_t)G.host_block_row.size(); break;
    case GMG_SSOR_PLAN_ROW_CI: src = G.w_row_ci.get(); len = 4 * L.n; break;
    case GMG_SSOR_PLAN_CI_ROW: src = G.w_ci_row.get(); len = 4 * G.w_n_coupled; break;
    case GMG_SSOR_PLAN_RPOS_F: src = G.w_rpos_f.get(); len = 4 * G.w_n_coupled; break;
    case GMG_SSOR_PLAN_RPOS_B: src = G.w_rpos_b.get(); len = 4 * G.w_n_coupled; break;
    case GMG_SSOR_PLAN_ISO_DIAG: src = G.w_iso_diag.get(); len = 8 * L.n; break;
    case GMG_SSOR_PLAN_ISO_INVD: src = G.w_iso_invd.get(); len = 8 * L.n; break;
    default: return fail(ctx, GMG_ERR_INVALID, "gmg_get_ssor_plan_array: unknown array");
  }
  if (!out) { *bytes = len; return GMG_OK; }
  if (*bytes < len) return fail(ctx, GMG_ERR_INVALID, "gmg_get_ssor_plan_array: the buffer is too small");
  *bytes = len;
  (void)hipSetDevice(ctx->device);
  if (len) HIPC(hipMemcpyAsync(out, src, (size_t)len, hipMemcpyDeviceToHost, ctx->stream));
  HIPC(hipStreamSynchronize(ctx->stream));
  return GMG_OK;
}

int gmg_get_ssor_plan_origin(gmg_context *ctx, int level, int *on_device, int64_t *csr_bytes_downloaded, const char **reason) {
  if (!ctx || level < 1 || level >= ctx->n_levels) return GMG_ERR_INVALID;
  const SgsPlan &G = ctx->lv[(size_t)level].sgs;
  if (G.host_block_row.empty()) return fail(ctx, GMG_ERR_INVALID, "gmg_get_ssor_plan_origin: the level matrix has not been set");
  if (on_device) *on_device = G.on_device ? 1 : 0;
  if (csr_bytes_downloaded) *csr_bytes_downloaded = G.csr_bytes_down;
  if (reason) *reason = G.host_reason;
  return GMG_OK;
}

int gmg_ssor_slot_plan(int64_t n, const int64_t *rowptr, const int32_t *col, const double *val, int64_t row_begin, int64_t row_end, int backward,
                       int32_t *step, int32_t *last_reader, int32_t *slot, int64_t *n_steps, int64_t *n_slots) {
  if (n < 0 || n > INT32_MAX || row_begin < 0 || row_end < row_begin || row_end > n || (n > 0 && (!rowptr || !col || !val)) || (n > 0 && rowptr[0] != 0)) return GMG_ERR_INVALID;
  for (int64_t i = 0; i < n; ++i) {
    if (rowptr[i + 1] < rowptr[i]) return GMG_ERR_INVALID;
    for (int64_t k = rowptr[i]; k < rowptr[i + 1]; ++k)
      if (col[k] < 0 || col[k] >= n) return GMG_ERR_INVALID;
  }
  const int m = (int)(row_end - row_begin), dir = backward ? 1 : 0;
  SsorBlockGraph B;
  SsorSlotPlan S;
  std::vector<int32_t> seq;
  std::vector<SsorStep> steps;
  if (m > 0) {
    if (!ssor_block_graph(row_begin, row_end, rowptr, col, val, B)) return GMG_ERR_INVALID;
    ssor_build_steps(dir, B.n_stages, B.sptr, B.by_stage, B.prp, B.pcol, kPhMaxRows, true, 0, kPhYSlots, seq, steps);
    ssor_slot_alloc(m, B.prp, B.pcol, dir, seq, steps, S);
  }
  if (step) std::copy(S.step.begin(), S.step.end(), step);
  if (last_reader) std::copy(S.last.begin(), S.last.end(), last_reader);
  if (slot) std::copy(S.slot.begin(), S.slot.end(), slot);
  if (n_steps) *n_steps = (int64_t)steps.size();
  if (n_slots) *n_slots = S.n_slots;
  return GMG_OK;
}

}
```

geometric-multigrid-preconditioners-for-long-range-coulomb-interaction_amd/csrc/gmg_sgs_layout.hpp:

```cpp
#pragma once
#include <stdint.h>

#include <algorithm>
#include <atomic>
#include <chrono>
#include <cstring>
#include <queue>
#include <vector>

#include "gmg_layout.hpp"

#ifdef __HIPCC__
#define GMG_HD __host__ __device__
#else
#define GMG_HD
#endif

namespace gmg {

constexpr int kSwRing = 32768;
constexpr int kSwChunk = 4096;
constexpr int kSwW = 32;
constexpr int kSwMaxBlock = 8192;
constexpr int kSwYSlots = 15744;
// ... 7 lines not shown
  int32_t n_ws;
  int32_t backward;
  int32_t first_raw, first_nrows, groups, pad1;
};
struct SwStepHdr {
  uint16_t nrows, flags;
  uint16_t next_nrows, pad;
  uint32_t advance;
  uint32_t next_raw;
};
GMG_HD constexpr int sw_stride(int g) { return 96 * g + 48; }

constexpr int kPhRegion = 16384;
constexpr int kPhMaxRows = 32;
constexpr int kPhMaxEntries = 36;
constexpr int kPhWaves = 4;
constexpr int kPhThreads = 64 * (kPhWaves + 1);
constexpr int kPhJunk = 512;
constexpr int kPhYSlots = (160 * 1024 - kPhWaves * kPhRegion - kPhJunk) / 8 & ~1;
GMG_HD constexpr bool ph_shape_ok(int g, int l1, int l2) {
  return g >= 0 && g <= 3 && l1 >= 4 && l1 <= 28 && l1 % 4 == 0 && l2 >= 0 && l2 <= 24 && l2 % 8 == 0 && 8 * g + l1 + l2 <= kPhMaxEntries;
}
GMG_HD constexpr int ph_stride(int g, int l) {
  const int s = 32 + 96 * g + 12 * l;
  return (s / 16) % 2 ? s : s + 16;
}
namespace ph {
GMG_HD constexpr int ph_key(int g, int l1, int l2) { return g * 64 + (l1 / 4) * 8 + l2 / 8; }
}

struct PhRange {
  int64_t stream_off;
  int32_t n_steps, ws_off, n_own, n_ws, backward, G, L;
  uint32_t blk_tab, L1;
  int32_t own_ci0, own_dir, pad0[2];
  uint32_t pf_lead, pf_step;
  uint32_t stream_bytes, pad;
};
struct PhBlkEntry { uint32_t off, bytes, word, pad; };

constexpr int kDpLate = 3;
constexpr int kDpPrep = 3;
constexpr int kDpSlots = 4;
constexpr int kDpThreads = 64 * (1 + kDpPrep);
constexpr int kDpMaxL1 = 28;
constexpr int kDpMaxL2 = 24;
GMG_HD constexpr int dp_cstride(int l1, int l2) {
  const int s = 48 + 12 * l1 + 8 * l2;
  return (s / 16) % 2 ? s : s + 16;
}
constexpr int kDpMaxStride = dp_cstride(28, 8);
static_assert(dp_cstride(12, 24) <= kDpMaxStride && dp_cstride(20, 16) <= kDpMaxStride && dp_cstride(24, 8) <= kDpMaxStride && dp_cstride(16, 16) <= kDpMaxStride, "slot size");
constexpr int kDpSlotBytes = 16 + kPhMaxRows * kDpMaxStride;
constexpr int kDpFlagBytes = 64;
constexpr int kDpYSlots = ((160 * 1024 - kDpSlots * ((kDpSlotBytes + 15) / 16 * 16) - kDpFlagBytes) / 8) & ~1;
constexpr int kRgYSlots = (160 * 1024 - kPhJunk) / 8 & ~1;

namespace sp {
GMG_HD inline bool fits(int ne, int first, int last, int g, int l1, int l2, int *h0o, int *h1o) {
  const int a = last + 1, b = ne - l2;
  const int h1 = a < b ? b : a;
  const int c = first < 8 * g ? first : 8 * g, d = h1 - l1;
  const int h0 = c < d ? d : c;
  if (h0 > first || h0 > 8 * g || h0 < 0) return false;
  if (h0o) { *h0o = h0; *h1o = h1; }
  return true;
}
GMG_HD inline double dmax(double a, double b) { return a < b ? b : a; }
GMG_HD inline double shape_cost(int g, int l1, int l2, double rows) {
  const int ent = 8 * g + l1 + l2;
  const double crit = 330.0 + 15.0 * l1 + 4.0 * l2, copy = 45.0 * (16.0 + rows * ph_stride(g, l1 + l2)) / 1024.0,
               p1 = 150.0 + 8.0 * (2.0 + 0.75 * ent), p2 = 100.0 + 11.0 * (8 * g + l2);
  return dmax(dmax(crit, copy), dmax(p1, p2)) + 0.1 * (crit + copy + p1 + p2);
}
GMG_HD inline void key_shape(int key, int *g, int *l1, int *l2) { *g = key >> 6; *l1 = 4 * (key >> 3 & 7); *l2 = 8 * (key & 7); }
}

struct SsorPlanOptions {
  bool disable_wave = false, disable_phase = false, profile = false, dep = false, reg = false, chain = false, sliding = true;
  int y_slots = 0, groups = 0, phase_chunk = 0;
  bool phase_nosplit = false, phase_nocascade = false;
  int pf_lead_kb = 0;
  bool debug = false;
};

constexpr double kSsorStepNs = 240.0;
constexpr double kSsorBytesPerNs = 48.0;
constexpr int64_t kSsorRowBytes = 64, kSsorEntryBytes = 28;

struct SsorPattern {
  int64_t n = 0;
  std::vector<int64_t> rp, trp;
  std::vector<int32_t> col, tcol;
  SsorPattern(int64_t n_, const int64_t *rp_, const int32_t *col_, const double *val) : n(n_) {
    rp.assign((size_t)n + 1, 0);
    for (int64_t i = 0; i < n; ++i) {
      for (int64_t k = rp_[i]; k < rp_[i + 1]; ++k)
        if (!val || val[k] != 0.0) col.push_back(col_[k]);
      rp[(size_t)i + 1] = (int64_t)col.size();
    }
    std::vector<double> ones(col.size(), 1.0), tval;
    transpose_host(n, n, rp.data(), col.data(), ones.data(), trp, tcol, tval);
  }
};

struct SsorBlockModel {
  const SsorPattern &P;
  std::vector<int32_t> stage, ent;
  std::vector<char> coupled;
  std::vector<int64_t> cnt;
  int64_t rb = 0, steps = 0, bytes = 0;
  explicit SsorBlockModel(const SsorPattern &p) : P(p), stage((size_t)p.n, 0), ent((size_t)p.n, 0), coupled((size_t)p.n, 0) {}
  void reset(int64_t r) { rb = r; steps = bytes = 0; cnt.clear(); }
  double cost_ns() const { return kSsorStepNs * (double)steps + (double)bytes / kSsorBytesPerNs; }
  void put(int32_t s) {
    if ((size_t)s >= cnt.size()) cnt.resize((size_t)s + 1, 0);
    if (cnt[(size_t)s]++ % kPhMaxRows == 0) steps += 2;
  }
  void add(int64_t i) {
    int32_t st = 0;
    bool low = false;
    auto touch = [&](int64_t j) {
      low = true;
      if (!coupled[(size_t)j]) {
        coupled[(size_t)j] = 1; stage[(size_t)j] = 0; put(0);
        bytes += kSsorRowBytes + kSsorEntryBytes * ent[(size_t)j];
      }
      st = std::max(st, stage[(size_t)j] + 1);
    };
    int32_t e = 0;
    for (int64_t k = P.rp[(size_t)i]; k < P.rp[(size_t)i + 1]; ++k) {
      const int64_t c = P.col[(size_t)k];
      if (c < rb || c > i) continue;
      ++e;
      if (c < i) touch(c);
    }
    for (int64_t k = P.trp[(size_t)i]; k < P.trp[(size_t)i + 1]; ++k) {
      const int64_t j = P.tcol[(size_t)k];
      if (j < rb || j >= i) continue;
      ent[(size_t)j]++;
      if (coupled[(size_t)j]) bytes += kSsorEntryBytes;
      touch(j);
    }
    ent[(size_t)i] = e;
    coupled[(size_t)i] = low;
    stage[(size_t)i] = low ? st : 0;
    if (low) { put(st); bytes += kSsorRowBytes + kSsorEntryBytes * e; }
  }
};

inline void ssor_balance(const SsorPattern &P, int n_blocks, std::vector<int64_t> &block_row, std::vector<double> &cost_us) {
  const int64_t n = P.n;
  const int nb = (int)std::max<int64_t>(1, std::min<int64_t>(n_blocks, (n + 63) / 64));
  SsorBlockModel M(P);
  auto greedy = [&](double T, std::vector<int64_t> *cuts) {
    int count = 1;
    M.reset(0);
    for (int64_t i = 0; i < n; ++i) {
      M.add(i);
      if (M.cost_ns() > T && i > M.rb) {
        if (++count > nb) return count;
        if (cuts) cuts->push_back(i);
        M.reset(i);
        M.add(i);
      }
    }
    return count;
  };
  M.reset(0);
  for (int64_t i = 0; i < n; ++i) M.add(i);
  double lo = 0.0, hi = M.cost_ns();
  while (hi - lo > 1e-4 * hi) {
    const double mid = 0.5 * (lo + hi);
    if (greedy(mid, nullptr) <= nb) hi = mid;
    else lo = mid;
  }
  std::vector<int64_t> cuts;
  greedy(hi, &cuts);
  block_row.assign((size_t)n_blocks + 1, n);
  block_row[0] = 0;
  for (size_t c = 0; c < cuts.size(); ++c) block_row[c + 1] = cuts[c];
  cost_us.assign((size_t)n_blocks, 0.0);
  for (int b = 0; b < n_blocks; ++b) {
    M.reset(block_row[(size_t)b]);
    for (int64_t i = block_row[(size_t)b]; i < block_row[(size_t)b + 1]; ++i) M.add(i);
    cost_us[(size_t)b] = M.cost_ns() * 1e-3;
  }
}

inline std::vector<double> ssor_block_costs(const SsorPattern &P, const std::vector<int32_t> &block_row) {
  SsorBlockModel M(P);
  std::vector<double> c(block_row.size() - 1, 0.0);
  for (size_t b = 0; b + 1 < block_row.size(); ++b) {
    M.reset(block_row[b]);
    for (int64_t i = block_row[b]; i < block_row[b + 1]; ++i) M.add(i);
    c[b] = M.cost_ns() * 1e-3;
  }
  return c;
}

struct SsorBlockGraph {
  std::vector<int32_t> prp, pcol, stage, crow, sptr, by_stage;
  std::vector<double> pval;
  std::vector<char> coupled;
  int n_stages = 0;
};
inline bool ssor_block_graph(int64_t rb, int64_t re, const int64_t *rp, const int32_t *col, const double *val, SsorBlockGraph &B) {
  const int m = (int)(re - rb);
  B.prp.assign((size_t)m + 1, 0); B.pcol.clear(); B.pval.clear();
  B.coupled.assign((size_t)m, 0);
  std::vector<int32_t> low_cnt((size_t)m + 1, 0);
  for (int i = 0; i < m; ++i) {
    for (int64_t k = rp[rb + i]; k < rp[rb + i + 1]; ++k) {
      const int64_t c = col[k];
      if (k > rp[rb + i] && c <= col[k - 1]) return false;
      if (c < rb || c >= re || val[k] == 0.0) continue;
      B.pcol.push_back((int32_t)(c - rb));
      B.pval.push_back(val[k]);
      if (c != rb + i) {
        B.coupled[(size_t)i] = 1; B.coupled[(size_t)(c - rb)] = 1;
        low_cnt[(size_t)std::max<int64_t>(i, c - rb) + 1]++;
      }
    }
    B.prp[(size_t)i + 1] = (int32_t)B.pcol.size();
  }
  for (int i = 0; i < m; ++i) low_cnt[(size_t)i + 1] += low_cnt[(size_t)i];
  std::vector<int32_t> low((size_t)low_cnt[(size_t)m]), fill(low_cnt.begin(), low_cnt.end() - 1);
  for (int i = 0; i < m; ++i)
    for (int32_t k = B.prp[(size_t)i]; k < B.prp[(size_t)i + 1]; ++k)
      if (B.pcol[(size_t)k] != i) low[(size_t)fill[(size_t)std::max(i, B.pcol[(size_t)k])]++] = std::min(i, B.pcol[(size_t)k]);
  B.stage.assign((size_t)m, 0);
  B.n_stages = 0;
  B.crow.clear();
  for (int i = 0; i < m; ++i) {
    if (!B.coupled[(size_t)i]) continue;
    int st = 0;
    for (int32_t k = low_cnt[(size_t)i]; k < low_cnt[(size_t)i + 1]; ++k) st = std::max(st, B.stage[(size_t)low[(size_t)k]] + 1);
    B.stage[(size_t)i] = st;
    B.n_stages = std::max(B.n_stages, st + 1);
    B.crow.push_back(i);
  }
  B.sptr.assign((size_t)B.n_stages + 1, 0);
  B.by_stage.assign(B.crow.size(), 0);
  for (int32_t i : B.crow) B.sptr[(size_t)B.stage[(size_t)i] + 1]++;
  for (int t = 0; t < B.n_stages; ++t) B.sptr[(size_t)t + 1] += B.sptr[(size_t)t];
  if (B.n_stages > 0) {
    std::vector<int32_t> pos(B.sptr.begin(), B.sptr.end() - 1);
    for (int32_t i : B.crow) B.by_stage[(size_t)pos[(size_t)B.stage[(size_t)i]]++] = i;
  }
  return true;
}

struct SsorStep { int32_t first, nrows, len; };

inline int ssor_dir_entries(const std::vector<int32_t> &prp, const std::vector<int32_t> &pcol, int dir, int i) {
  int c = 0;
  for (int32_t k = prp[(size_t)i]; k < prp[(size_t)i + 1]; ++k) c += dir == 0 ? pcol[(size_t)k] < i : pcol[(size_t)k] >= i;
  return c;
}

inline void ssor_build_steps(int dir, int n_stages, const std::vector<int32_t> &sptr, const std::vector<int32_t> &by_stage, const std::vector<int32_t> &prp,
                      const std::vector<int32_t> &pcol, int max_rows, bool ph, int stride, int y_cap, std::vector<int32_t> &seq, std::vector<SsorStep> &steps) {
  seq.clear(); steps.clear();
  seq.reserve(by_stage.size());
  for (int t = 0; t < n_stages; ++t) {
    const int tt = dir == 0 ? t : n_stages - 1 - t;
    SsorStep cur{(int32_t)seq.size(), 0, 0};
    for (int32_t qq = sptr[(size_t)tt]; qq < sptr[(size_t)tt + 1]; ++qq) {
      const int32_t q = dir == 0 ? qq : sptr[(size_t)tt] + sptr[(size_t)tt + 1] - 1 - qq;
      const int i = by_stage[(size_t)q];
      const int li = ssor_dir_entries(prp, pcol, dir, i);
      const int nl = std::max(cur.len, li);
      const int64_t raw = 16 + (int64_t)(cur.nrows + 1) * stride;
      if (cur.nrows > 0 && (cur.nrows == max_rows || (!ph && raw > kSwMaxBlock) || (cur.nrows + 1) * (nl + 1) > y_cap)) {
        steps.push_back(cur);
        cur = SsorStep{(int32_t)seq.size(), 0, 0};
      }
      cur.len = std::max(cur.len, li);
      cur.nrows++;
      seq.push_back(i);
    }
    if (cur.nrows) steps.push_back(cur);
  }
}

struct SsorSlotPlan {
  std::vector<int32_t> step, last, slot;
  int n_slots = 0;
};
inline void ssor_slot_alloc(int m, const std::vector<int32_t> &prp, const std::vector<int32_t> &pcol, int dir, const std::vector<int32_t> &seq,
                     const std::vector<SsorStep> &steps, SsorSlotPlan &out) {
  out.step.assign((size_t)m, -1); out.last.assign((size_t)m, -1); out.slot.assign((size_t)m, -1);
  out.n_slots = 0;
  for (size_t s = 0; s < steps.size(); ++s)
    for (int u = 0; u < steps[s].nrows; ++u) out.step[(size_t)seq[(size_t)(steps[s].first + u)]] = (int32_t)s;
  for (int32_t i : seq) {
    out.last[(size_t)i] = std::max(out.last[(size_t)i], out.step[(size_t)i]);
    for (int32_t k = prp[(size_t)i]; k < prp[(size_t)i + 1]; ++k) {
      const int c = pcol[(size_t)k];
      if (dir == 0 ? c < i : c > i) out.last[(size_t)c] = std::max(out.last[(size_t)c], out.step[(size_t)i]);
    }
  }
  const int hold = 2;
  std::vector<std::vector<int32_t>> due(steps.size() + 1);
  std::priority_queue<int32_t, std::vector<int32_t>, std::greater<int32_t>> free_slots;
  for (size_t s = 0; s < steps.size(); ++s) {
    for (int32_t i : due[s]) free_slots.push(out.slot[(size_t)i]);
    for (int u = 0; u < steps[s].nrows; ++u) {
      const int i = seq[(size_t)(steps[s].first + u)];
      if (free_slots.empty()) out.slot[(size_t)i] = out.n_slots++;
      else { out.slot[(size_t)i] = free_slots.top(); free_slots.pop(); }
      const size_t rel = (size_t)out.last[(size_t)i] + (size_t)hold;
      if (rel < steps.size()) due[rel].push_back(i);
    }
  }
}

inline std::vector<int32_t> ssor_block_rows(int64_t n, const int64_t *rp, const int32_t *col, const double *val, const std::vector<int64_t> *explicit_rows,
                                            bool balanced, int blocks) {
  if (explicit_rows) return std::vector<int32_t>(explicit_rows->begin(), explicit_rows->end());
  const int nb = (int)std::max<int64_t>(1, std::min<int64_t>(blocks, (n + 63) / 64));
  std::vector<int32_t> block_row((size_t)nb + 1);
  if (balanced) {
    std::vector<int64_t> br;
    std::vector<double> cost;
    ssor_balance(SsorPattern(n, rp, col, val), nb, br, cost);
    block_row.assign(br.begin(), br.end());
  } else {
    for (int b = 0; b <= nb; ++b) block_row[(size_t)b] = (int32_t)(n * b / nb);
  }
  return block_row;
}

struct SsorGenericPlan {
  std::vector<int32_t> stage_ptr, stage_rows, block_stage;
  int n_stages_max = 0;
};
inline SsorGenericPlan ssor_generic_plan(int64_t n, const int64_t *rp, const int32_t *col, const std::vector<int32_t> &block_row) {
  std::vector<int64_t> trp;
  std::vector<int32_t> tcol;
  std::vector<double> tval, ones((size_t)rp[n], 1.0);
  transpose_host(n, n, rp, col, ones.data(), trp, tcol, tval);
  const int n_blocks = (int)block_row.size() - 1;
  SsorGenericPlan G;
  G.block_stage.assign((size_t)n_blocks + 1, 0);
  G.stage_rows.resize((size_t)std::max<int64_t>(n, 1));
  std::vector<int32_t> stage((size_t)std::max<int64_t>(n, 1), 0);
  for (int b = 0; b < n_blocks; ++b) {
    const int64_t rb = block_row[(size_t)b], re = block_row[(size_t)b + 1];
    int ns = 0;
    for (int64_t i = rb; i < re; ++i) {
      int s = 0;
      for (int64_t k = rp[i]; k < rp[i + 1]; ++k)
        if (col[k] < i && col[k] >= rb) s = std::max(s, stage[(size_t)col[k]] + 1);
      for (int64_t k = trp[(size_t)i]; k < trp[(size_t)i + 1]; ++k)
        if (tcol[(size_t)k] < i && tcol[(size_t)k] >= rb) s = std::max(s, stage[(size_t)tcol[(size_t)k]] + 1);
      stage[(size_t)i] = s;
      ns = std::max(ns, s + 1);
    }
    if (re == rb) ns = 0;
    std::vector<int32_t> cnt((size_t)ns + 1, 0);
    for (int64_t i = rb; i < re; ++i) cnt[(size_t)stage[(size_t)i] + 1]++;
    for (int t = 0; t < ns; ++t) cnt[(size_t)t + 1] += cnt[(size_t)t];
    std::vector<int32_t> pos(cnt.begin(), cnt.end());
    for (int64_t i = rb; i < re; ++i) G.stage_rows[(size_t)(rb + pos[(size_t)stage[(size_t)i]]++)] = (int32_t)i;
    for (int t = 0; t <= ns; ++t) G.stage_ptr.push_back((int32_t)(rb + cnt[(size_t)t]));
    G.block_stage[(size_t)b + 1] = G.block_stage[(size_t)b] + ns;
    G.n_stages_max = std::max(G.n_stages_max, ns);
  }
  return G;
}

enum SsorOutcome {
  kSsorPlanned,
  kSsorGeneric,
  kSsorOneWave,
  kSsorUnsupported,
  kSsorInvalid
};
struct SsorSweepPlan {
  SsorOutcome outcome = kSsorPlanned;
  const char *message = "";
  bool phased = false, dep = false, reg = false;
  std::vector<SwRange> ranges;
  std::vector<PhRange> pranges;
  std::vector<PhBlkEntry> blk_tab;
  std::vector<int32_t> block_rng, ws_ci, ci_row, row_ci, rpos_f, rpos_b;
  std::vector<char> stream;
  std::vector<double> iso_diag, iso_invd;
  std::vector<int32_t> bwd_rows;
  std::vector<int64_t> block_steps, block_bytes;
  int y_slots = 0, lds_bytes = 0, n_self = 0, live_max[2] = {0, 0}, n_bwd = 0;
  int64_t total_steps = 0, total_stages = 0;
  std::vector<int64_t> hist_g = std::vector<int64_t>(4, 0), hist_l1 = std::vector<int64_t>(8, 0), hist_l2 = std::vector<int64_t>(4, 0);
  double laps[4] = {0, 0, 0, 0};
  int n_ranges() const { return (int)(phased ? pranges.size() : ranges.size()); }
};

struct SsorRowCut { int32_t ne, first, last; };
struct SsorShape { int g, l1, l2; };

inline SsorShape ssor_choose_shape(const SsorPlanOptions &opt, bool dep, bool reg, const std::vector<SsorRowCut> &cut, size_t u0, size_t u1, double rows) {
  double best = 1e300;
  SsorShape bs{-1, 0, 0};
  for (int g = 0; g <= 3; ++g)
    for (int l1 = 4; l1 <= 28; l1 += 4)
      for (int l2 = 0; l2 <= 24; l2 += 8) {
        if (!ph_shape_ok(g, l1, l2) || (opt.phase_nosplit && l2 > 0) || (dep && l1 > kDpMaxL1)) continue;
        bool ok = true;
        for (size_t u = u0; u < u1 && ok; ++u) ok = sp::fits(cut[u].ne, cut[u].first, cut[u].last, g, l1, l2, nullptr, nullptr);
        if (!ok) continue;
        double cost;
        if (dep) {
          cost = 20.0 * l1 + 8.0 * l2 + 2.0 * g;
        } else if (reg) {
          const double crit = 330.0 + 15.0 * l1 + 4.0 * l2, p2 = 100.0 + 11.0 * (8 * g + l2), load = 60.0 + 20.0 * (2.0 + 6.0 * g + 0.75 * (l1 + l2));
          cost = std::max(std::max(crit, load), p2) + 0.1 * (crit + load + p2);
        } else {
          cost = sp::shape_cost(g, l1, l2, rows);
        }
        if (cost < best) { best = cost; bs = SsorShape{g, l1, l2}; }
      }
  return bs;
}

struct SsorSweepBuilder {
  const SsorPlanOptions &opt;
  SsorSweepPlan &P;
  bool ph = false, dep = false, reg = false, fieldmajor = false, slide_ok = false;
  int late_steps = 1, y_max = 0, y_cap = 0, max_ws = 0;
  std::chrono::steady_clock::time_point lap_t = std::chrono::steady_clock::now();
  int64_t rb = 0;
  SsorBlockGraph B;
  std::vector<int32_t> ws_stamp, own_stamp, tmp_stamp, upd_stamp, slot_of, step_of, prefix_pos;
  int stamp_id = 0, tmp_id = 0;
  std::vector<SwRange> dir_ranges[2];
  std::vector<PhRange> dir_pranges[2];
  int dir = 0;
  std::vector<int32_t> seq;
  std::vector<SsorStep> steps;

  SsorSweepBuilder(const SsorPlanOptions &o, SsorSweepPlan &p) : opt(o), P(p) {}
  void lap(int k) {
    const auto t = std::chrono::steady_clock::now();
    P.laps[k] += std::chrono::duration<double>(t - lap_t).count();
    lap_t = t;
  }
  bool stop(SsorOutcome o, const char *why) { P.outcome = o; P.message = why; return false; }
  template <class F>
  void for_rows(size_t s0, size_t s1, F f) const {
    for (size_t st = s0; st < s1; ++st)
      for (int u = 0; u < steps[st].nrows; ++u) f((int32_t)(st - s0), (int)seq[(size_t)(steps[st].first + u)]);
  }
  template <class F>
  void for_entries(int i, F f) const {
    for (int32_t k = B.prp[(size_t)i]; k < B.prp[(size_t)i + 1]; ++k)
      if (dir == 0 ? B.pcol[(size_t)k] < i : B.pcol[(size_t)k] >= i) f(k, (int)B.pcol[(size_t)k]);
  }

  int choose_groups() const {
    if (opt.groups > 0) return std::min(4, opt.groups);
    std::vector<int> stage_len((size_t)B.n_stages, 0);
    for (int32_t i : B.crow) stage_len[(size_t)B.stage[(size_t)i]] = std::max(stage_len[(size_t)B.stage[(size_t)i]], ssor_dir_entries(B.prp, B.pcol, dir, i));
    int g_dir = 2;
    double best = 1e300;
    for (int gg = 1; gg <= 4; ++gg) {
      double cost = 0;
      for (int t = 0; t < B.n_stages; ++t) cost += (double)std::max(1, (stage_len[(size_t)t] + 8 * gg - 1) / (8 * gg)) * (3.0 + gg);
      if (cost < best) { best = cost; g_dir = gg; }
    }
    return g_dir;
  }

  size_t greedy_range(size_t s0, SwRange &R) {
    size_t s1 = s0;
    int ws = 0;
    while (s1 < steps.size()) {
      ++tmp_id;
      int add = 0;
      auto count = [&](int r) {
        if (ws_stamp[(size_t)r] != stamp_id && tmp_stamp[(size_t)r] != tmp_id) { tmp_stamp[(size_t)r] = tmp_id; ++add; }
      };
      for_rows(s1, s1 + 1, [&](int32_t, int i) { count(i); for_entries(i, [&](int32_t, int c) { count(c); }); });
      if (ws + add > y_cap) {
        if (s1 > s0) break;
        return s0;
      }
      ws += add;
      for_rows(s1, s1 + 1, [&](int32_t, int i) { ws_stamp[(size_t)i] = stamp_id; for_entries(i, [&](int32_t, int c) { ws_stamp[(size_t)c] = stamp_id; }); });
      ++s1;
    }
    int n_slot = 0;
    auto take = [&](int r) {
      own_stamp[(size_t)r] = stamp_id;
      slot_of[(size_t)r] = n_slot++;
      P.ws_ci.push_back(P.row_ci[(size_t)(rb + r)]);
    };
    for_rows(s0, s1, [&](int32_t, int i) { take(i); });
    R.n_own = n_slot;
    for_rows(s0, s1, [&](int32_t, int i) { for_entries(i, [&](int32_t, int c) { if (own_stamp[(size_t)c] != stamp_id) take(c); }); });
    R.n_ws = n_slot;
    max_ws = std::max(max_ws, n_slot);
    return s1;
  }

  std::vector<SsorRowCut> row_cuts(size_t s0, size_t s1) const {
    std::vector<SsorRowCut> cut;
    for_rows(s0, s1, [&](int32_t st, int i) {
      int ne = 0, first_late = -1, last_late = -1;
      for_entries(i, [&](int32_t, int c) {
        if (c != i && upd_stamp[(size_t)c] == stamp_id && step_of[(size_t)c] >= st - late_steps && step_of[(size_t)c] < st) {
          if (first_late < 0) first_late = ne;
// ... 122 lines not shown
    prefetch(R4, off);
    P.total_steps += R4.n_steps;
    dir_pranges[dir].push_back(R4);
    lap(3);
    return true;
  }

  bool wave_range(size_t s0, size_t s1, SwRange &R, int g) {
    const int w_dir = 8 * g, stride = sw_stride(g);
    const int64_t base = ((int64_t)P.stream.size() + kSwChunk - 1) / kSwChunk * kSwChunk;
    R.stream_off = base;
    int64_t off = 0, prev_hdr = -1;
    auto link = [&](uint32_t next_raw, int next_nrows) {
      SwStepHdr h;
      std::memcpy(&h, P.stream.data() + base + prev_hdr, sizeof h);
      h.advance = (uint32_t)(off - prev_hdr); h.next_raw = next_raw;
      if (next_raw) h.next_nrows = (uint16_t)next_nrows;
      std::memcpy(P.stream.data() + base + prev_hdr, &h, sizeof h);
    };
    for (size_t st = s0; st < s1; ++st) {
      const SsorStep &S = steps[st];
      const int nr = S.nrows, n_sub = std::max(1, (S.len + w_dir - 1) / w_dir);
      for (int sub = 0; sub < n_sub; ++sub) {
        const int64_t raw = 16 + (int64_t)nr * stride;
        if (off % kSwRing + raw > kSwRing) off = (off / kSwRing + 1) * kSwRing;
        P.stream.resize((size_t)(base + off + raw), 0);
        char *blk = P.stream.data() + base + off;
        SwStepHdr h{};
        h.nrows = (uint16_t)nr;
        h.flags = (uint16_t)((sub == 0 ? 1 : 0) | (sub == n_sub - 1 ? 2 : 0));
        std::memcpy(blk, &h, sizeof h);
        if (prev_hdr >= 0) link((uint32_t)raw, nr);
        else { R.first_raw = (int32_t)raw; R.first_nrows = nr; }
        prev_hdr = off;
        for (int u = 0; u < nr; ++u) {
          const int i = seq[(size_t)(S.first + u)];
          const int32_t ci = P.row_ci[(size_t)(rb + i)];
          char *rec = blk + 16 + (size_t)u * stride;
          const int64_t rec_pos = base + off + 16 + (int64_t)u * stride;
          if (sub == n_sub - 1) (dir == 0 ? P.rpos_f : P.rpos_b)[(size_t)ci] = (int32_t)(rec_pos / 8);
          if (dir == 1 && sub == 0) prefix_pos[(size_t)i] = (int32_t)(rec_pos / 8 + 2);
          double *f = reinterpret_cast<double *>(rec);
          uint32_t *w = reinterpret_cast<uint32_t *>(rec);
          const uint32_t my = (uint32_t)slot_of[(size_t)i] * 8u;
          f[0] = 0.0; f[1] = P.iso_invd[(size_t)(rb + i)]; f[2] = 0.0;
          w[6] = my;
          w[7] = dir == 0 ? (uint32_t)prefix_pos[(size_t)i] : 0u;
          uint32_t *ad = reinterpret_cast<uint32_t *>(rec + 32 + 64 * g);
          int e = 0, seen = 0;
          for_entries(i, [&](int32_t k, int c) {
            if (seen++ < sub * w_dir || e >= 8 * g) return;
            f[4 + e] = B.pval[(size_t)k];
            ad[e++] = (uint32_t)slot_of[(size_t)c] * 8u;
          });
          for (; e < 8 * g; ++e) { f[4 + e] = 0.0; ad[e] = my; }
        }
        off += raw;
        R.n_steps++;
      }
    }
    if (prev_hdr >= 0) link(0, 0);
    const int64_t padded = (off + kSwChunk - 1) / kSwChunk * kSwChunk;
    if (padded >= ((int64_t)1 << 31) || (base + padded) / 8 >= ((int64_t)1 << 31)) return stop(kSsorGeneric, "stream positions beyond 2^31");
    P.stream.resize((size_t)(base + padded), 0);
    R.stream_bytes = (int32_t)padded;
    P.total_steps += R.n_steps;
    dir_ranges[dir].push_back(R);
    return true;
  }

  bool block(int64_t rb_, int64_t re, const int64_t *rp, const int32_t *col, const double *val) {
    rb = rb_;
    const int m = (int)(re - rb);
    if (!ssor_block_graph(rb, re, rp, col, val, B)) return stop(kSsorGeneric, "unsorted columns");
    for (int64_t i = rb; i < re; ++i)
      for (int64_t k = rp[i]; k < rp[i + 1]; ++k)
        if (col[k] == i) { P.iso_diag[(size_t)i] = val[k]; P.iso_invd[(size_t)i] = 1.0 / val[k]; }
    lap(0);
    const size_t ci_base = P.ci_row.size();
    P.ci_row.resize(ci_base + B.crow.size());
    P.rpos_f.resize(P.ci_row.size(), 0);
    P.rpos_b.resize(P.ci_row.size(), 0);
    if (B.crow.empty()) return true;
    P.total_stages += B.n_stages;
    for (size_t q = 0; q < B.by_stage.size(); ++q) {
      P.row_ci[(size_t)(rb + B.by_stage[q])] = (int32_t)(ci_base + q);
      P.ci_row[ci_base + q] = (int32_t)(rb + B.by_stage[q]);
    }
    for (std::vector<int32_t> *v : {&ws_stamp, &own_stamp, &tmp_stamp, &upd_stamp, &step_of}) v->assign((size_t)m, -1);
    slot_of.assign((size_t)m, 0); prefix_pos.assign((size_t)m, 0);
    stamp_id = tmp_id = 0;
    for (int d = 0; d < 2; ++d) { dir_ranges[d].clear(); dir_pranges[d].clear(); }
    SsorSlotPlan slide[2];
    std::vector<int32_t> slide_seq[2];
    std::vector<SsorStep> slide_steps[2];
    bool sliding = slide_ok;
    for (int d = 0; d < 2 && slide_ok; ++d) {
      ssor_build_steps(d, B.n_stages, B.sptr, B.by_stage, B.prp, B.pcol, kPhMaxRows, true, 0, y_max, slide_seq[d], slide_steps[d]);
      ssor_slot_alloc(m, B.prp, B.pcol, d, slide_seq[d], slide_steps[d], slide[d]);
      P.live_max[d] = std::max(P.live_max[d], slide[d].n_slots);
      if (((slide[d].n_slots + 1) & ~1) > y_cap) sliding = false;
    }
    lap(1);
    for (dir = 1; dir >= 0; --dir) {
      const int g_dir = choose_groups();
      if (sliding) { seq.swap(slide_seq[dir]); steps.swap(slide_steps[dir]); }
      else ssor_build_steps(dir, B.n_stages, B.sptr, B.by_stage, B.prp, B.pcol, ph ? kPhMaxRows : 64, ph, ph ? ph_stride(3, 12) : sw_stride(g_dir), y_cap, seq, steps);
      for (size_t s0 = 0, s1 = 0; s0 < steps.size(); s0 = s1) {
        ++stamp_id;
        SwRange R{};
        R.ws_off = (int32_t)P.ws_ci.size();
        R.backward = dir;
        R.groups = g_dir;
        if (sliding) {
          s1 = steps.size();
          for (int32_t i : seq) slot_of[(size_t)i] = slide[dir].slot[(size_t)i];
          max_ws = std::max(max_ws, slide[dir].n_slots);
        } else {
          s1 = greedy_range(s0, R);
          if (s1 == s0) return stop(kSsorUnsupported, "SGS plan: one step exceeds the LDS working set");
        }
        if (!(ph ? phase_range(s0, s1, R, sliding, slide[dir].n_slots) : wave_range(s0, s1, R, g_dir))) return false;
      }
    }
    dir = 0;
    for (int d = 0; d < 2; ++d) P.ranges.insert(P.ranges.end(), dir_ranges[d].begin(), dir_ranges[d].end());
    for (int d = 0; d < 2; ++d) P.pranges.insert(P.pranges.end(), dir_pranges[d].begin(), dir_pranges[d].end());
    return true;
  }
};

inline void ssor_sweep_plan(const SsorPlanOptions &opt, int64_t n, const int64_t *rp, const int32_t *col, const double *val,
                            const std::vector<int32_t> &block_row, bool allow_phase, SsorSweepPlan &P) {
  P = SsorSweepPlan();
  SsorSweepBuilder S(opt, P);
  if (n <= 0 || opt.disable_wave) { S.stop(kSsorGeneric, n <= 0 ? "empty level" : "wave disabled"); return; }
  const int n_blocks = (int)block_row.size() - 1;
  bool ph = allow_phase && !opt.disable_phase && !opt.profile;
  for (int64_t i = 0; i < n && ph; ++i) ph = rp[i + 1] - rp[i] <= 2 * kPhMaxEntries;
  S.ph = P.phased = ph;
  S.dep = P.dep = ph && opt.dep;
  S.reg = P.reg = ph && !S.dep && opt.reg && !opt.chain;
  S.fieldmajor = S.dep || S.reg;
  S.slide_ok = ph && !S.dep && !S.reg && !opt.chain && opt.sliding;
  S.late_steps = S.dep ? kDpLate : 1;
  S.y_max = S.dep ? kDpYSlots : S.reg ? kRgYSlots : ph ? kPhYSlots : kSwYSlots;
  S.y_cap = std::max(64, std::min(opt.y_slots > 0 ? opt.y_slots : S.y_max, S.y_max)) & ~1;
  P.row_ci.assign((size_t)n, -1);
  P.block_rng.assign((size_t)n_blocks + 1, 0);
  P.iso_diag.assign((size_t)n, 0.0); P.iso_invd.assign((size_t)n, 1.0);
  P.block_steps.assign((size_t)n_blocks, 0); P.block_bytes.assign((size_t)n_blocks, 0);
  for (int b = 0; b < n_blocks; ++b) {
    const int64_t steps0 = P.total_steps, bytes0 = (int64_t)P.stream.size();
    P.block_rng[(size_t)b] = P.n_ranges();
    if (block_row[(size_t)b + 1] > block_row[(size_t)b] && !S.block(block_row[(size_t)b], block_row[(size_t)b + 1], rp, col, val)) return;
    P.block_steps[(size_t)b] = P.total_steps - steps0; P.block_bytes[(size_t)b] = (int64_t)P.stream.size() - bytes0;
  }
  P.block_rng[(size_t)n_blocks] = P.n_ranges();
  P.y_slots = std::max(2, (S.max_ws + 1) & ~1);
  P.lds_bytes = P.dep   ? P.y_slots * 8 + kDpSlots * ((kDpSlotBytes + 15) / 16 * 16) + kDpFlagBytes
                : P.reg ? P.y_slots * 8 + kPhJunk
                : ph    ? P.y_slots * 8 + kPhWaves * kPhRegion + kPhJunk
                        : P.y_slots * 8 + kSwRing + 32;
  for (const PhRange &R : P.pranges) P.n_bwd += R.backward;
  for (const SwRange &R : P.ranges) P.n_bwd += R.backward;
  S.lap(3);
}

inline const char *check_sweep_plan(const SsorSweepPlan &P, int64_t n) {
  static const char *const bad_rec = "SSOR plan: a record addresses memory outside the stream / the LDS slots (internal error)",
                    *const bad_bwd = "SSOR plan: a backward record stores outside the level vector (internal error)";
  const uint64_t size = P.stream.size(), lds = (uint64_t)P.y_slots * 8;
  std::atomic<bool> ok{true}, ok_bwd{true};
  auto record = [&](auto unit, int ad_off, int n_ad, bool backward, bool self) {
    const uint32_t my = *reinterpret_cast<const uint32_t *>(unit(24)), aux = *reinterpret_cast<const uint32_t *>(unit(28));
    bool good = (uint64_t)my + 8 <= lds && (backward || (uint64_t)aux * 8 + 8 <= size);
    for (int e = 0; e < n_ad; ++e) good = good && (uint64_t)*reinterpret_cast<const uint32_t *>(unit(ad_off + 4 * e)) + 8 <= lds;
    if (!good) ok = false;
    if (backward && self && aux >= (uint64_t)n) ok_bwd = false;
  };
  for (const PhRange &R : P.pranges) {
    if (R.n_steps < 0 || R.stream_off < 0 || (size_t)R.blk_tab + (size_t)R.n_steps > P.blk_tab.size()) return bad_rec;
    parallel_chunks(R.n_steps, [&](int64_t q0, int64_t q1, int) {
      for (int64_t q = q0; q < q1; ++q) {
        const PhBlkEntry &e = P.blk_tab[(size_t)R.blk_tab + (size_t)q];
        int g, l1, l2;
        sp::key_shape((int)(e.word & 255u), &g, &l1, &l2);
        const int nrows = (int)(e.word >> 8 & 255u), stride = ph_stride(g, l1 + l2);
        if (!ph_shape_ok(g, l1, l2) || (uint64_t)R.stream_off + e.off + 16 + (uint64_t)nrows * stride > size) { ok = false; continue; }
        const char *blk = P.stream.data() + R.stream_off + e.off;
        for (int u = 0; u < nrows; ++u)
          record([&](int o) { return P.dep || P.reg ? blk + 16 + ((size_t)(o / 16) * nrows + u) * 16 + o % 16 : blk + 16 + (size_t)u * stride + o; },
                 32 + 64 * g + 8 * (l1 + l2), 8 * g + l1 + l2, R.backward != 0, R.pad0[0] == 1);
      }
    });
  }
  for (const SwRange &R : P.ranges) {
    int64_t pos = R.stream_off;
    for (int s = 0; s < R.n_steps; ++s) {
      if (pos < 0 || (uint64_t)pos + 16 > size) return bad_rec;
      SwStepHdr h;
      std::memcpy(&h, P.stream.data() + pos, sizeof h);
      if (R.groups < 1 || R.groups > 4 || (uint64_t)pos + 16 + (uint64_t)h.nrows * sw_stride(R.groups) > size) return bad_rec;
      for (int u = 0; u < h.nrows; ++u)
        record([&](int o) { return P.stream.data() + pos + 16 + (size_t)u * sw_stride(R.groups) + o; }, 32 + 64 * R.groups, 8 * R.groups, R.backward != 0, false);
      pos += h.advance;
    }
  }
  if (!ok) return bad_rec;
  for (int32_t r : P.bwd_rows) ok_bwd = ok_bwd && r >= 0 && r < n;
  if (!ok_bwd) return bad_bwd;
  for (int32_t ci : P.ws_ci)
    if (ci < 0 || (size_t)ci >= P.ci_row.size()) return "SSOR plan: working-set entry out of range (internal error)";
  for (size_t q = 0; q < P.rpos_f.size(); ++q)
    if ((uint64_t)P.rpos_f[q] * 8 + 8 > size || (uint64_t)P.rpos_b[q] * 8 + 8 > size) return "SSOR plan: rhs position outside the stream (internal error)";
  return nullptr;
}

}
```

include/gmg_coulomb.h:

```cpp
#ifndef GMG_COULOMB_H
#define GMG_COULOMB_H

#include <stdint.h>

#ifdef __cplusplus
extern "C" {
#endif

#define GMG_OK 0
#define GMG_ERR_INVALID 1
#define GMG_ERR_OUTER_NOCONV 2
#define GMG_ERR_COARSE_NOCONV 3
#define GMG_ERR_HIP 4
#define GMG_ERR_COMM 5
#define GMG_ERR_UNSUPPORTED 6

#define GMG_SYSTEM (-1)

#define GMG_SMOOTHER_JACOBI 0
#define GMG_SMOOTHER_SSOR 1
#define GMG_SMOOTHER_CHEBYSHEV 2

#define GMG_PRECOND_GMG 0
#define GMG_PRECOND_JACOBI 1
// ... 179 lines not shown
                       double *residual_sq, double *face_int, double *threshold, uint8_t *mark, int64_t *n_marked,
                       double *build_ms);

int gmg_build_face_table_resident(gmg_context *ctx, int dim, const int32_t n0[3], int n_levels, const int64_t *level_ptr,
                                  const int32_t *cell_coord, const int32_t *cell_first_child, int64_t *n_active, double *build_ms);
int gmg_get_face_table(gmg_context *ctx, int64_t *n_active, uint8_t *face_kind, int32_t *face_cell);
int gmg_estimate_error_resident(gmg_context *ctx, const double *h_of_level, const double *face_measure_of_level,
                                const double *diameter_of_level, int ng, const double *gauss_x, const double *gauss_w, const double *u,
                                int64_t n_u, int residual, int nq, const double *weight, const double *jxw_of_level, const double *dens,
                                double fraction, float *eta, double *kelly_sq, double *residual_sq, double *face_int, double *threshold,
                                uint8_t *mark, int64_t *n_marked, double *build_ms);
int gmg_get_marks(gmg_context *ctx, int64_t *n_cells, uint8_t *mark, int64_t *n_marked);
int gmg_refine_forest_marked(gmg_context *ctx, int dim, const int32_t n0[3], int n_levels, const int64_t *level_ptr,
                             const int32_t *cell_coord, const int32_t *cell_first_child, int *new_n_levels, int64_t *new_n_cells,
                             int64_t *n_split, double *build_ms);
int gmg_energy_norm_error_resident(gmg_context *ctx, double origin, double h0, const double *u, int64_t n_u, int64_t n_atoms,
                                   const double *atom_xyz, const double *atom_q, double r_c, int nq, const double *quadrature_points,
                                   const double *weights, const double *shape_grad, double *error, double *cell_err2);

int gmg_build_point_locator_resident(gmg_context *ctx, int dim, const int32_t n0[3], int n_levels, const int64_t *level_ptr,
                                     const int32_t *cell_coord, const int32_t *cell_first_child, int64_t *n_nodes, double *build_ms);
int gmg_get_point_locator(gmg_context *ctx, int64_t *n_nodes, int32_t *node);
int gmg_atom_forces_resident(gmg_context *ctx, double origin, double h0, int64_t n_atoms, const double *atom_xyz, const double *atom_q,
                             const double *u, int64_t n_u, double r_c, double cutoff, double *phi, double *field, double *force,
                             double *force_short, double *e_short);
int gmg_electrostatic_energy_resident(gmg_context *ctx, double origin, double h0, int64_t n_atoms, const double *atom_xyz,
                                      const double *atom_q, const double *u, int64_t n_u, double r_c, double cutoff, double out[3],
                                      double *build_ms);

typedef struct gmg_stats {
  int64_t coarse_solves;
  int64_t coarse_iterations;
  int64_t vcycles;
  int64_t spmv0_samples;
  double spmv0_ms_total;
  int64_t spmv0_rows, spmv0_nnz;
  int64_t cgupd_samples;
  double cgupd_ms_total;
  int64_t coarse_variant;
  int64_t spmv0_layout;
  int64_t spmv0_matrix_bytes;
  int64_t spmv0_pattern_slices, spmv0_slices;
  int64_t coarse_enqueued;
  int64_t spmv0_noop_samples;
  double spmv0_noop_ms_total;
  int64_t sgs_samples;
  double sgs_ms_total;
  int64_t sgs_substeps;
  int64_t sgs_stream_bytes;
  int64_t sgs_launches;
  double build_matrices_ms;
  int64_t coarse_solver;
} gmg_stats;
int gmg_stats_reset(gmg_context *ctx);
int gmg_stats_get(gmg_context *ctx, gmg_stats *out);
int gmg_set_profiling(gmg_context *ctx, int sample_every);
int gmg_calibrate_hbm(gmg_context *ctx, int64_t n_bytes, int reps, double *read_gbps, double *copy_gbps);
int gmg_set_tuning(gmg_context *ctx, int coarse_chunk, int cg_variant);
int gmg_set_option(gmg_context *ctx, const char *key, double value);
int gmg_set_ssor_blocks(gmg_context *ctx, int n_blocks);
#define GMG_SSOR_PARTITION_ROWS 0
#define GMG_SSOR_PARTITION_BALANCED 1
int gmg_set_ssor_block_rows(gmg_context *ctx, int level, int n_blocks, const int64_t *block_row);
int gmg_set_ssor_partition(gmg_context *ctx, int kind);
int gmg_get_ssor_partition(gmg_context *ctx, int level, int *n_blocks, int64_t *block_row, int64_t *block_steps);
int gmg_ssor_balance_rows(int64_t n, const int64_t *rowptr, const int32_t *col, const double *val, int n_blocks,
                          int64_t *block_row, double *block_cost);
int gmg_get_ssor_plan(gmg_context *ctx, int level, int64_t out[8]);
int gmg_get_ssor_backward_rows(gmg_context *ctx, int level, int64_t *count, int32_t *rows);
#define GMG_SSOR_PLAN_STREAM 0
#define GMG_SSOR_PLAN_RANGES 1
#define GMG_SSOR_PLAN_BLK_TAB 2
#define GMG_SSOR_PLAN_BLOCK_RNG 3
#define GMG_SSOR_PLAN_ROW_CI 4
#define GMG_SSOR_PLAN_CI_ROW 5
#define GMG_SSOR_PLAN_RPOS_F 6
#define GMG_SSOR_PLAN_RPOS_B 7
#define GMG_SSOR_PLAN_ISO_DIAG 8
#define GMG_SSOR_PLAN_ISO_INVD 9
int gmg_get_ssor_plan_array(gmg_context *ctx, int level, int which, int64_t *bytes, void *out);
int gmg_get_ssor_plan_origin(gmg_context *ctx, int level, int *on_device, int64_t *csr_bytes_downloaded, const char **reason);
int gmg_ssor_slot_plan(int64_t n, const int64_t *rowptr, const int32_t *col, const double *val, int64_t row_begin, int64_t row_end,
                       int backward, int32_t *step, int32_t *last_reader, int32_t *slot, int64_t *n_steps, int64_t *n_slots);

#ifdef __cplusplus
}
#endif
#endif
```

Measured before the change: 151.8 million.

## Pack SSOR sweep rows into dense critical-path levels to cut sub-steps

Adds a list-scheduling pass that reassigns coupled rows of each SSOR block to levels of up to kPhMaxRows rows, prioritised by dependency-chain height. This replaces the original stage grouping, so the sliding-window sweep runs fewer, fuller sequential sub-steps. It is enabled by default for levels of at least 8192 rows, and falls back to the old stages if the y slots or shapes don't fit. Such levels now build their SSOR plan on the host instead of the device, which adds setup cost.

Measured after the change: 159.2 million, median of 6. 4.9% higher.

```diff
diff --git a/geometric-multigrid-preconditioners-for-long-range-coulomb-interaction_amd/capi.py b/geometric-multigrid-preconditioners-for-long-range-coulomb-interaction_amd/capi.py
--- a/geometric-multigrid-preconditioners-for-long-range-coulomb-interaction_amd/capi.py
+++ b/geometric-multigrid-preconditioners-for-long-range-coulomb-interaction_amd/capi.py
@@ -49,6 +49,7 @@
     "gmg_gaussian_potential", "gmg_energy_norm_error",
     "gmg_get_ssor_plan", "gmg_get_ssor_backward_rows", "gmg_ssor_slot_plan",
     "gmg_get_ssor_plan_array", "gmg_get_ssor_plan_origin",
+    "gmg_ssor_pack_levels", "gmg_ssor_slot_plan_packed", "gmg_get_ssor_schedule",
 ]
 
 
@@ -1004,6 +1005,11 @@
         self._chk(self.L.gmg_get_ssor_plan(self.h, C.c_int(level), _p(out, C.c_int64)))
         return dict(zip(SSOR_PLAN_KEYS, (int(v) for v in out)))
 
+    def get_ssor_schedule(self, level):
+        out = np.zeros(4, dtype=np.int64)
+        self._chk(self.L.gmg_get_ssor_schedule(self.h, C.c_int(level), _p(out, C.c_int64)))
+        return dict(zip(SSOR_SCHEDULE_KEYS, (int(v) for v in out)))
+
     def get_ssor_backward_rows(self, level):
         cnt = C.c_int64(0)
         self._chk(self.L.gmg_get_ssor_backward_rows(self.h, C.c_int(level), C.byref(cnt), None))
@@ -1027,20 +1033,35 @@
 
 SSOR_PLAN_ARRAYS = ("stream", "ranges", "blk_tab", "block_rng", "row_ci", "ci_row", "rpos_f", "rpos_b", "iso_diag", "iso_invd")
 SSOR_PLAN_KEYS = ("forward_ranges", "backward_ranges", "self_contained_ranges", "y_slots", "max_live_forward", "max_live_backward", "steps", "stream_bytes")
-
-
-def ssor_slot_plan(m, row_begin, row_end, backward):
+SSOR_SCHEDULE_KEYS = ("packed", "levels", "steps_per_direction", "stage_steps")
+
+
+def ssor_slot_plan(m, row_begin, row_end, backward, packed=False):
     rp, col, val = _csr(m)
     n = len(rp) - 1
     k = max(int(row_end) - int(row_begin), 1)
     step, last, slot = (np.full(k, -1, dtype=np.int32) for _ in range(3))
     ns, nl = C.c_int64(0), C.c_int64(0)
-    rc = load().gmg_ssor_slot_plan(C.c_int64(n), _p(rp, C.c_int64), _p(col, C.c_int32), _p(val, C.c_double), C.c_int64(int(row_begin)), C.c_int64(int(row_end)),
-                                   C.c_int(int(bool(backward))), _p(step, C.c_int32), _p(last, C.c_int32), _p(slot, C.c_int32), C.byref(ns), C.byref(nl))
+    name = "gmg_ssor_slot_plan_packed" if packed else "gmg_ssor_slot_plan"
+    rc = getattr(load(), name)(C.c_int64(n), _p(rp, C.c_int64), _p(col, C.c_int32), _p(val, C.c_double), C.c_int64(int(row_begin)), C.c_int64(int(row_end)),
+                               C.c_int(int(bool(backward))), _p(step, C.c_int32), _p(last, C.c_int32), _p(slot, C.c_int32), C.byref(ns), C.byref(nl))
     if rc != OK:
-        raise GMGError(rc, "gmg_ssor_slot_plan")
+        raise GMGError(rc, name)
     k = int(row_end) - int(row_begin)
     return step[:k], last[:k], slot[:k], ns.value, nl.value
+
+
+def ssor_pack_levels(m, row_begin, row_end):
+    rp, col, val = _csr(m)
+    n = len(rp) - 1
+    k = int(row_end) - int(row_begin)
+    level = np.full(max(k, 1), -1, dtype=np.int32)
+    nl, ns = C.c_int64(0), C.c_int64(0)
+    rc = load().gmg_ssor_pack_levels(C.c_int64(n), _p(rp, C.c_int64), _p(col, C.c_int32), _p(val, C.c_double), C.c_int64(int(row_begin)), C.c_int64(int(row_end)),
+                                     _p(level, C.c_int32), C.byref(nl), C.byref(ns))
+    if rc != OK:
+        raise GMGError(rc, "gmg_ssor_pack_levels")
+    return level[:k], nl.value, ns.value
 
 
 def ssor_balance_rows(m, n_blocks, use_values=True):
diff --git a/geometric-multigrid-preconditioners-for-long-range-coulomb-interaction_amd/csrc/gmg_coulomb.hip b/geometric-multigrid-preconditioners-for-long-range-coulomb-interaction_amd/csrc/gmg_coulomb.hip
--- a/geometric-multigrid-preconditioners-for-long-range-coulomb-interaction_amd/csrc/gmg_coulomb.hip
+++ b/geometric-multigrid-preconditioners-for-long-range-coulomb-interaction_amd/csrc/gmg_coulomb.hip
@@ -106,6 +106,8 @@
   std::vector<int32_t> host_bwd_rows;
   int n_self = 0, live_max[2] = {0, 0};
   int64_t w_n_coupled = 0, w_stream_bytes = 0, w_steps = 0, w_stages = 0;
+  int n_packed = 0;
+  int64_t w_fwd_steps = 0, w_stage_steps = 0;
   std::vector<int32_t> host_block_row;
   std::vector<int64_t> host_block_steps;
   std::vector<int64_t> host_block_bytes;
@@ -261,6 +263,7 @@
   int sgs_y_slots = 0;
   bool ssor_plan_device = false;
   bool sgs_sliding = true;
+  int sgs_pack = -1;
   bool sgs_disable_wave = false, sgs_disable_phase = false, sgs_chain = false, sgs_dep = false, sgs_reg = false, debug_upload = false, sgs_profile = false;
   int sgs_profile_mode = 0;
   int sgs_phase_chunk = 0;
@@ -1385,7 +1388,7 @@
   o.dep = ctx->sgs_dep; o.reg = ctx->sgs_reg; o.chain = ctx->sgs_chain; o.sliding = ctx->sgs_sliding;
   o.y_slots = ctx->sgs_y_slots; o.groups = ctx->sgs_groups; o.phase_chunk = ctx->sgs_phase_chunk;
   o.phase_nosplit = ctx->sgs_phase_nosplit; o.phase_nocascade = ctx->sgs_phase_nocascade; o.pf_lead_kb = ctx->sgs_pf_lead_kb;
-  o.debug = ctx->debug_upload;
+  o.debug = ctx->debug_upload; o.pack = ctx->sgs_pack;
   return o;
 }
 
@@ -1398,6 +1401,7 @@
   G.w_y_slots = W.y_slots; G.w_lds_bytes = W.lds_bytes; G.w_n_ranges = W.n_ranges(); G.n_bwd = W.n_bwd;
   G.phased = W.phased; G.dep = W.dep; G.reg = W.reg;
   G.w_n_coupled = n_coupled; G.w_stream_bytes = stream_bytes; G.w_steps = W.total_steps; G.w_stages = W.total_stages;
+  G.n_packed = W.n_packed; G.w_fwd_steps = W.fwd_steps; G.w_stage_steps = W.stage_steps;
 }
 
 void sgs_plan_log(const SgsPlan &G, const SsorSweepPlan &W, int64_t n) {
@@ -1407,9 +1411,12 @@
                  (long long)hist_g[2], (long long)hist_g[3], (long long)hist_l1[0], (long long)hist_l1[1], (long long)hist_l1[2], (long long)hist_l1[3], (long long)hist_l1[4],
                  (long long)hist_l1[5], (long long)hist_l1[6], (long long)hist_l1[7], (long long)hist_l2[0], (long long)hist_l2[1], (long long)hist_l2[2], (long long)hist_l2[3]);
   std::fprintf(stderr, "[gmg] SGS %s plan: %lld rows, %lld coupled, %d blocks, %lld stages, %lld sub-steps, %d ranges (%d forward + %d backward, %d self-contained), "
-               "y slots %d (most live: forward %d, backward %d), stream %.1f MB\n",
+               "y slots %d (most live: forward %d, backward %d), stream %.1f MB; schedule: packed %d, levels %lld, steps per direction %lld, by stages %lld "
+               "(blocks kept on their stages: %d for the y slots, %d for a step without a shape)\n",
                W.phased ? "four-wave" : "one-wave", (long long)n, (long long)G.w_n_coupled, (int)G.host_block_row.size() - 1, (long long)G.w_stages, (long long)G.w_steps, G.w_n_ranges,
-               G.w_n_ranges - G.n_bwd, G.n_bwd, G.n_self, G.w_y_slots, G.live_max[0], G.live_max[1], (double)G.w_stream_bytes / 1e6);
+               G.w_n_ranges - G.n_bwd, G.n_bwd, G.n_self, G.w_y_slots, G.live_max[0], G.live_max[1], (double)G.w_stream_bytes / 1e6,
+               G.n_packed > 0 ? 1 : 0, (long long)G.w_stages, (long long)G.w_fwd_steps, (long long)G.w_stage_steps,
+               W.n_pack_no_slots, W.n_pack_no_shape);
 }
 
 void sgs_partition_log(gmg_context *ctx, Level &L, int64_t n, const int64_t *rp, const int32_t *col, const double *val, const std::vector<int32_t> &block_row,
@@ -1502,7 +1509,7 @@
   return dim3((unsigned)g);
 }
 
-const char *sgs_device_refusal(const gmg_context *ctx, bool explicit_rows) {
+const char *sgs_device_refusal(const gmg_context *ctx, bool explicit_rows, int64_t n) {
   if (ctx->dist) return "communicator";
   if (!explicit_rows && ctx->ssor_partition == GMG_SSOR_PARTITION_BALANCED) return "balanced partition";
   if (!ctx->sgs_sliding) return "option sgs_sliding unset";
@@ -1517,12 +1524,13 @@
   if (ctx->sgs_phase_nosplit) return "option sgs_phase_nosplit set";
   if (ctx->sgs_phase_nocascade) return "option sgs_phase_nocascade set";
   if (ctx->sgs_pf_lead_kb) return "option sgs_pf_lead_kb set";
+  if (ssor_pack_wanted(ssor_plan_options(ctx), n)) return "packed schedule";
   return nullptr;
 }
 
 int setup_sgs_device(gmg_context *ctx, Level &L, int64_t n, const int32_t *rp, const int32_t *col, const double *val,
                      const std::vector<int64_t> *explicit_rows, const char **reason) {
-  *reason = sgs_device_refusal(ctx, explicit_rows != nullptr);
+  *reason = sgs_device_refusal(ctx, explicit_rows != nullptr, n);
   if (*reason) return GMG_OK;
   if (n <= 0) { *reason = "empty level"; return GMG_OK; }
   const std::vector<int32_t> block_row = ssor_block_rows(n, nullptr, nullptr, nullptr, explicit_rows, false, ctx->ssor_blocks);
@@ -1736,6 +1744,7 @@
   W.y_slots = y_slots;
   W.lds_bytes = y_slots * 8 + kPhWaves * kPhRegion + kPhJunk;
   W.total_steps = n_steps; W.total_stages = total_stages;
+  W.fwd_steps = W.stage_steps = n_steps / 2;
   sgs_set_host_members(G, W, block_row, nct, stream_size);
   G.on_device = true;
   CHK(sgs_wave_tail(ctx, G, true, false, false));
@@ -2115,7 +2124,7 @@
     if (ctx->ssor_plan_device) {
       DevPtr<int32_t> d_rp, d_col;
       DevPtr<double> d_val;
-      if (!sgs_device_refusal(ctx, explicit_rows != nullptr) && n_rows > 0) {
+      if (!sgs_device_refusal(ctx, explicit_rows != nullptr, n_rows) && n_rows > 0) {
         if (rowptr[n_rows] > INT32_MAX) return fail(ctx, GMG_ERR_INVALID, "gmg_set_level_matrix: more than 2^31 entries");
         const std::vector<int32_t> rp32(rowptr, rowptr + n_rows + 1);
         HIPC(upload(d_rp, rp32, ctx->stream));
@@ -5101,6 +5110,7 @@
   else if (k == "ssor_balanced") ctx->ssor_partition = on ? GMG_SSOR_PARTITION_BALANCED : GMG_SSOR_PARTITION_ROWS;
   else if (k == "sgs_y_slots") ctx->sgs_y_slots = (int)value;
   else if (k == "sgs_sliding") ctx->sgs_sliding = on;
+  else if (k == "sgs_pack") ctx->sgs_pack = value < 0 ? -1 : on ? 1 : 0;
   else if (k == "ssor_plan_device") ctx->ssor_plan_device = on;
   else if (k == "sgs_disable_wave") ctx->sgs_disable_wave = on;
   else if (k == "sgs_disable_phase") ctx->sgs_disable_phase = on;
@@ -5253,6 +5263,16 @@
   if (!G.wave) return GMG_OK;
   out[0] = G.w_n_ranges - G.n_bwd; out[1] = G.n_bwd; out[2] = G.n_self; out[3] = G.w_y_slots;
   out[4] = G.live_max[0]; out[5] = G.live_max[1]; out[6] = G.w_steps; out[7] = G.w_stream_bytes;
+  return GMG_OK;
+}
+
+int gmg_get_ssor_schedule(gmg_context *ctx, int level, int64_t out[4]) {
+  if (!ctx || !out || level < 1 || level >= ctx->n_levels) return GMG_ERR_INVALID;
+  const SgsPlan &G = ctx->lv[(size_t)level].sgs;
+  if (G.host_block_row.empty()) return fail(ctx, GMG_ERR_INVALID, "gmg_get_ssor_schedule: the level matrix has not been set");
+  std::fill(out, out + 4, (int64_t)0);
+  if (!G.wave) return GMG_OK;
+  out[0] = G.n_packed > 0 ? 1 : 0; out[1] = G.w_stages; out[2] = G.w_fwd_steps; out[3] = G.w_stage_steps;
   return GMG_OK;
 }
 
@@ -5330,4 +5350,54 @@
   return GMG_OK;
 }
 
-}
+static bool ssor_host_csr_ok(int64_t n, const int64_t *rowptr, const int32_t *col, const double *val, int64_t row_begin, int64_t row_end) {
+  if (n < 0 || n > INT32_MAX || row_begin < 0 || row_end < row_begin || row_end > n || (n > 0 && (!rowptr || !col || !val)) || (n > 0 && rowptr[0] != 0)) return false;
+  for (int64_t i = 0; i < n; ++i) {
+    if (rowptr[i + 1] < rowptr[i]) return false;
+    for (int64_t k = rowptr[i]; k < rowptr[i + 1]; ++k)
+      if (col[k] < 0 || col[k] >= n) return false;
+  }
+  return true;
+}
+
+int gmg_ssor_pack_levels(int64_t n, const int64_t *rowptr, const int32_t *col, const double *val, int64_t row_begin, int64_t row_end, int32_t *level,
+                         int64_t *n_levels, int64_t *n_stage_steps) {
+  if (!ssor_host_csr_ok(n, rowptr, col, val, row_begin, row_end)) return GMG_ERR_INVALID;
+  SsorBlockGraph B;
+  SsorLevels Lv;
+  if (row_end > row_begin) {
+    if (!ssor_block_graph(row_begin, row_end, rowptr, col, val, B)) return GMG_ERR_INVALID;
+    ssor_pack_levels(B, Lv);
+    for (size_t i = 0; i < Lv.level.size(); ++i)
+      if (!B.coupled[i]) Lv.level[i] = -1;
+  }
+  if (level) std::copy(Lv.level.begin(), Lv.level.end(), level);
+  if (n_levels) *n_levels = Lv.n_levels;
+  if (n_stage_steps) *n_stage_steps = Lv.stage_steps;
+  return GMG_OK;
+}
+
+int gmg_ssor_slot_plan_packed(int64_t n, const int64_t *rowptr, const int32_t *col, const double *val, int64_t row_begin, int64_t row_end, int backward,
+                              int32_t *step, int32_t *last_reader, int32_t *slot, int64_t *n_steps, int64_t *n_slots) {
+  if (!ssor_host_csr_ok(n, rowptr, col, val, row_begin, row_end)) return GMG_ERR_INVALID;
+  const int m = (int)(row_end - row_begin), dir = backward ? 1 : 0;
+  SsorBlockGraph B;
+  SsorLevels Lv;
+  SsorSlotPlan S;
+  std::vector<int32_t> seq;
+  std::vector<SsorStep> steps;
+  if (m > 0) {
+    if (!ssor_block_graph(row_begin, row_end, rowptr, col, val, B)) return GMG_ERR_INVALID;
+    ssor_pack_levels(B, Lv);
+    ssor_build_steps(dir, Lv.n_levels, Lv.sptr, Lv.by_level, B.prp, B.pcol, kPhMaxRows, true, 0, kPhYSlots, seq, steps);
+    ssor_slot_alloc(m, B.prp, B.pcol, dir, seq, steps, S);
+  }
+  if (step) std::copy(S.step.begin(), S.step.end(), step);
+  if (last_reader) std::copy(S.last.begin(), S.last.end(), last_reader);
+  if (slot) std::copy(S.slot.begin(), S.slot.end(), slot);
+  if (n_steps) *n_steps = (int64_t)steps.size();
+  if (n_slots) *n_slots = S.n_slots;
+  return GMG_OK;
+}
+
+}
diff --git a/geometric-multigrid-preconditioners-for-long-range-coulomb-interaction_amd/csrc/gmg_sgs_layout.hpp b/geometric-multigrid-preconditioners-for-long-range-coulomb-interaction_amd/csrc/gmg_sgs_layout.hpp
--- a/geometric-multigrid-preconditioners-for-long-range-coulomb-interaction_amd/csrc/gmg_sgs_layout.hpp
+++ b/geometric-multigrid-preconditioners-for-long-range-coulomb-interaction_amd/csrc/gmg_sgs_layout.hpp
@@ -113,7 +113,13 @@
   bool phase_nosplit = false, phase_nocascade = false;
   int pf_lead_kb = 0;
   bool debug = false;
-};
+  int pack = -1;
+};
+constexpr int64_t kPhPackMinRows = 8192;
+inline bool ssor_pack_wanted(const SsorPlanOptions &opt, int64_t n) {
+  const bool self = !opt.disable_wave && !opt.disable_phase && !opt.profile && !opt.dep && !opt.reg && !opt.chain && opt.sliding;
+  return self && (opt.pack > 0 || (opt.pack < 0 && n >= kPhPackMinRows));
+}
 
 constexpr double kSsorStepNs = 240.0;
 constexpr double kSsorBytesPerNs = 48.0;
@@ -236,6 +242,16 @@
   std::vector<char> coupled;
   int n_stages = 0;
 };
+inline void ssor_rows_by_stage(const std::vector<int32_t> &crow, const std::vector<int32_t> &stage, int n_stages, std::vector<int32_t> &sptr, std::vector<int32_t> &by_stage) {
+  sptr.assign((size_t)n_stages + 1, 0);
+  by_stage.assign(crow.size(), 0);
+  for (int32_t i : crow) sptr[(size_t)stage[(size_t)i] + 1]++;
+  for (int t = 0; t < n_stages; ++t) sptr[(size_t)t + 1] += sptr[(size_t)t];
+  if (n_stages > 0) {
+    std::vector<int32_t> pos(sptr.begin(), sptr.end() - 1);
+    for (int32_t i : crow) by_stage[(size_t)pos[(size_t)stage[(size_t)i]]++] = i;
+  }
+}
 inline bool ssor_block_graph(int64_t rb, int64_t re, const int64_t *rp, const int32_t *col, const double *val, SsorBlockGraph &B) {
   const int m = (int)(re - rb);
   B.prp.assign((size_t)m + 1, 0); B.pcol.clear(); B.pval.clear();
@@ -271,15 +287,53 @@
     B.n_stages = std::max(B.n_stages, st + 1);
     B.crow.push_back(i);
   }
-  B.sptr.assign((size_t)B.n_stages + 1, 0);
-  B.by_stage.assign(B.crow.size(), 0);
-  for (int32_t i : B.crow) B.sptr[(size_t)B.stage[(size_t)i] + 1]++;
-  for (int t = 0; t < B.n_stages; ++t) B.sptr[(size_t)t + 1] += B.sptr[(size_t)t];
-  if (B.n_stages > 0) {
-    std::vector<int32_t> pos(B.sptr.begin(), B.sptr.end() - 1);
-    for (int32_t i : B.crow) B.by_stage[(size_t)pos[(size_t)B.stage[(size_t)i]]++] = i;
-  }
+  ssor_rows_by_stage(B.crow, B.stage, B.n_stages, B.sptr, B.by_stage);
   return true;
+}
+
+struct SsorLevels {
+  std::vector<int32_t> level, sptr, by_level;
+  int n_levels = 0;
+  int64_t stage_steps = 0;
+};
+inline void ssor_pack_levels(const SsorBlockGraph &B, SsorLevels &Lv) {
+  const size_t m = B.stage.size();
+  Lv.level.assign(m, 0);
+  Lv.n_levels = 0;
+  Lv.stage_steps = 0;
+  for (int t = 0; t < B.n_stages; ++t) Lv.stage_steps += (B.sptr[(size_t)t + 1] - B.sptr[(size_t)t] + kPhMaxRows - 1) / kPhMaxRows;
+  std::vector<int32_t> up_ptr(m + 1, 0), n_low(m, 0), height(m, 0);
+  for (size_t i = 0; i < m; ++i)
+    for (int32_t k = B.prp[i]; k < B.prp[i + 1]; ++k)
+      if (B.pcol[(size_t)k] != (int32_t)i) {
+        up_ptr[(size_t)std::min<int32_t>((int32_t)i, B.pcol[(size_t)k]) + 1]++;
+        n_low[(size_t)std::max<int32_t>((int32_t)i, B.pcol[(size_t)k])]++;
+      }
+  for (size_t i = 0; i < m; ++i) up_ptr[i + 1] += up_ptr[i];
+  std::vector<int32_t> up((size_t)up_ptr[m]), fill(up_ptr.begin(), up_ptr.end() - 1);
+  for (size_t i = 0; i < m; ++i)
+    for (int32_t k = B.prp[i]; k < B.prp[i + 1]; ++k)
+      if (B.pcol[(size_t)k] != (int32_t)i) up[(size_t)fill[(size_t)std::min<int32_t>((int32_t)i, B.pcol[(size_t)k])]++] = std::max<int32_t>((int32_t)i, B.pcol[(size_t)k]);
+  for (size_t i = m; i-- > 0;)
+    for (int32_t k = up_ptr[i]; k < up_ptr[i + 1]; ++k) height[i] = std::max(height[i], height[(size_t)up[(size_t)k]] + 1);
+  auto key = [&](int32_t i) { return (uint64_t)(uint32_t)height[(size_t)i] << 32 | (uint32_t)~(uint32_t)i; };
+  std::priority_queue<uint64_t> ready;
+  for (int32_t i : B.crow)
+    if (n_low[(size_t)i] == 0) ready.push(key(i));
+  std::vector<int32_t> taken;
+  for (int t = 0; !ready.empty(); ++t) {
+    taken.clear();
+    while (!ready.empty() && (int)taken.size() < kPhMaxRows) {
+      taken.push_back((int32_t)~(uint32_t)(ready.top() & 0xffffffffu));
+      ready.pop();
+    }
+    for (int32_t i : taken) Lv.level[(size_t)i] = t;
+    for (int32_t i : taken)
+      for (int32_t k = up_ptr[(size_t)i]; k < up_ptr[(size_t)i + 1]; ++k)
+        if (--n_low[(size_t)up[(size_t)k]] == 0) ready.push(key(up[(size_t)k]));
+    Lv.n_levels = t + 1;
+  }
+  ssor_rows_by_stage(B.crow, Lv.level, Lv.n_levels, Lv.sptr, Lv.by_level);
 }
 
 struct SsorStep { int32_t first, nrows, len; };
@@ -423,6 +477,8 @@
   std::vector<int64_t> block_steps, block_bytes;
   int y_slots = 0, lds_bytes = 0, n_self = 0, live_max[2] = {0, 0}, n_bwd = 0;
   int64_t total_steps = 0, total_stages = 0;
+  int n_packed = 0, n_pack_no_slots = 0, n_pack_no_shape = 0;
+  int64_t fwd_steps = 0, stage_steps = 0;
   std::vector<int64_t> hist_g = std::vector<int64_t>(4, 0), hist_l1 = std::vector<int64_t>(8, 0), hist_l2 = std::vector<int64_t>(4, 0);
   double laps[4] = {0, 0, 0, 0};
   int n_ranges() const { return (int)(phased ? pranges.size() : ranges.size()); }
@@ -458,7 +514,7 @@
 struct SsorSweepBuilder {
   const SsorPlanOptions &opt;
   SsorSweepPlan &P;
-  bool ph = false, dep = false, reg = false, fieldmajor = false, slide_ok = false;
+  bool ph = false, dep = false, reg = false, fieldmajor = false, slide_ok = false, pack = false;
   int late_steps = 1, y_max = 0, y_cap = 0, max_ws = 0;
   std::chrono::steady_clock::time_point lap_t = std::chrono::steady_clock::now();
   int64_t rb = 0;
@@ -747,6 +803,51 @@
     P.rpos_f.resize(P.ci_row.size(), 0);
     P.rpos_b.resize(P.ci_row.size(), 0);
     if (B.crow.empty()) return true;
+    const int step_rows = ph ? kPhMaxRows : 64;
+    for (int t = 0; t < B.n_stages; ++t) P.stage_steps += (B.sptr[(size_t)t + 1] - B.sptr[(size_t)t] + step_rows - 1) / step_rows;
+    SsorSlotPlan slide[2];
+    std::vector<int32_t> slide_seq[2];
+    std::vector<SsorStep> slide_steps[2];
+    auto self_contained = [&]() {
+      bool fits = true;
+      for (int d = 0; d < 2; ++d) {
+        ssor_build_steps(d, B.n_stages, B.sptr, B.by_stage, B.prp, B.pcol, kPhMaxRows, true, 0, y_max, slide_seq[d], slide_steps[d]);
+        ssor_slot_alloc(m, B.prp, B.pcol, d, slide_seq[d], slide_steps[d], slide[d]);
+        if (((slide[d].n_slots + 1) & ~1) > y_cap) fits = false;
+      }
+      return fits;
+    };
+    auto shapes_exist = [&]() {
+      bool ok = true;
+      for (int d = 0; d < 2 && ok; ++d) {
+        dir = d;
+        seq.swap(slide_seq[d]); steps.swap(slide_steps[d]);
+        ++stamp_id;
+        for_rows(0, steps.size(), [&](int32_t st, int i) { step_of[(size_t)i] = st; upd_stamp[(size_t)i] = stamp_id; });
+        std::vector<SsorShape> shape_of;
+        ok = choose_shapes(0, steps.size(), row_cuts(0, steps.size()), shape_of);
+        seq.swap(slide_seq[d]); steps.swap(slide_steps[d]);
+      }
+      dir = 0;
+      return ok;
+    };
+    bool sliding = false, slots_known = false;
+    if (pack) {
+      SsorLevels Lv;
+      ssor_pack_levels(B, Lv);
+      auto exchange = [&]() { B.stage.swap(Lv.level); B.sptr.swap(Lv.sptr); B.by_stage.swap(Lv.by_level); std::swap(B.n_stages, Lv.n_levels); };
+      exchange();
+      for (std::vector<int32_t> *v : {&upd_stamp, &step_of}) v->assign((size_t)m, -1);
+      stamp_id = 0;
+      const bool fits = self_contained();
+      sliding = slots_known = fits && shapes_exist();
+      if (sliding) ++P.n_packed;
+      else { exchange(); ++(fits ? P.n_pack_no_shape : P.n_pack_no_slots); }
+    }
+    if (slide_ok && !slots_known) sliding = self_contained();
+    if (slide_ok)
+      for (int d = 0; d < 2; ++d) P.live_max[d] = std::max(P.live_max[d], slide[d].n_slots);
+    lap(1);
     P.total_stages += B.n_stages;
     for (size_t q = 0; q < B.by_stage.size(); ++q) {
       P.row_ci[(size_t)(rb + B.by_stage[q])] = (int32_t)(ci_base + q);
@@ -756,21 +857,11 @@
     slot_of.assign((size_t)m, 0); prefix_pos.assign((size_t)m, 0);
     stamp_id = tmp_id = 0;
     for (int d = 0; d < 2; ++d) { dir_ranges[d].clear(); dir_pranges[d].clear(); }
-    SsorSlotPlan slide[2];
-    std::vector<int32_t> slide_seq[2];
-    std::vector<SsorStep> slide_steps[2];
-    bool sliding = slide_ok;
-    for (int d = 0; d < 2 && slide_ok; ++d) {
-      ssor_build_steps(d, B.n_stages, B.sptr, B.by_stage, B.prp, B.pcol, kPhMaxRows, true, 0, y_max, slide_seq[d], slide_steps[d]);
-      ssor_slot_alloc(m, B.prp, B.pcol, d, slide_seq[d], slide_steps[d], slide[d]);
-      P.live_max[d] = std::max(P.live_max[d], slide[d].n_slots);
-      if (((slide[d].n_slots + 1) & ~1) > y_cap) sliding = false;
-    }
-    lap(1);
     for (dir = 1; dir >= 0; --dir) {
       const int g_dir = choose_groups();
       if (sliding) { seq.swap(slide_seq[dir]); steps.swap(slide_steps[dir]); }
       else ssor_build_steps(dir, B.n_stages, B.sptr, B.by_stage, B.prp, B.pcol, ph ? kPhMaxRows : 64, ph, ph ? ph_stride(3, 12) : sw_stride(g_dir), y_cap, seq, steps);
+      if (dir == 0) P.fwd_steps += (int64_t)steps.size();
       for (size_t s0 = 0, s1 = 0; s0 < steps.size(); s0 = s1) {
         ++stamp_id;
         SwRange R{};
@@ -808,6 +899,7 @@
   S.reg = P.reg = ph && !S.dep && opt.reg && !opt.chain;
   S.fieldmajor = S.dep || S.reg;
   S.slide_ok = ph && !S.dep && !S.reg && !opt.chain && opt.sliding;
+  S.pack = S.slide_ok && ssor_pack_wanted(opt, n);
   S.late_steps = S.dep ? kDpLate : 1;
   S.y_max = S.dep ? kDpYSlots : S.reg ? kRgYSlots : ph ? kPhYSlots : kSwYSlots;
   S.y_cap = std::max(64, std::min(opt.y_slots > 0 ? opt.y_slots : S.y_max, S.y_max)) & ~1;
diff --git a/include/gmg_coulomb.h b/include/gmg_coulomb.h
--- a/include/gmg_coulomb.h
+++ b/include/gmg_coulomb.h
@@ -285,6 +285,11 @@
 int gmg_get_ssor_plan_origin(gmg_context *ctx, int level, int *on_device, int64_t *csr_bytes_downloaded, const char **reason);
 int gmg_ssor_slot_plan(int64_t n, const int64_t *rowptr, const int32_t *col, const double *val, int64_t row_begin, int64_t row_end,
                        int backward, int32_t *step, int32_t *last_reader, int32_t *slot, int64_t *n_steps, int64_t *n_slots);
+int gmg_ssor_pack_levels(int64_t n, const int64_t *rowptr, const int32_t *col, const double *val, int64_t row_begin, int64_t row_end,
+                         int32_t *level, int64_t *n_levels, int64_t *n_stage_steps);
+int gmg_ssor_slot_plan_packed(int64_t n, const int64_t *rowptr, const int32_t *col, const double *val, int64_t row_begin, int64_t row_end,
+                              int backward, int32_t *step, int32_t *last_reader, int32_t *slot, int64_t *n_steps, int64_t *n_slots);
+int gmg_get_ssor_schedule(gmg_context *ctx, int level, int64_t out[4]);
 
 #ifdef __cplusplus
 }
```
